# tongdaxu/VQ-VAE-from-Gaussian-VAE

Measured on AMD Instinct MI355X. Metric: images/sec encode+quantize+decode, 256x256, codebook 2^16, higher is better.
Workload: dtype f32

## Files before the change

include/gqhip.h:

```cpp
#ifndef GQHIP_H_
#define GQHIP_H_

#include <stdint.h>

#ifdef __cplusplus
extern "C" {
#endif

#define GQHIP_ABI_VERSION 8

typedef int64_t gqhip_gnstat_t;
#define GQHIP_GNSTAT_WORDS 8

typedef enum gqhip_status {
  GQHIP_OK = 0,
  GQHIP_ERR_INVALID_ARG = 1,
  GQHIP_ERR_WORKSPACE = 2,
  GQHIP_ERR_LAUNCH = 3,
  GQHIP_ERR_NO_DEVICE = 4
} gqhip_status;

int gqhip_abi_version(void);
const char *gqhip_status_string(int status);
int gqhip_last_hip_error(void);

#define GQHIP_FILTER_AUTO 0
#define GQHIP_FILTER_FP32 1
#define GQHIP_FILTER_BF16 2
#define GQHIP_FILTER_MIXED 3
int gqhip_set_filter(int kind);
int gqhip_get_filter(void);

int gqhip_debug_plan(int64_t rows, int64_t n, int64_t dim, int64_t *out8);


int64_t gqhip_workspace_bytes(int64_t rows, int64_t n, int64_t dim);

int64_t gqhip_cb_cache_bytes(int64_t n, int64_t dim);
int gqhip_grid_search_applies(int64_t n, int64_t dim);
int gqhip_cb_cache_degenerate(const void *cb_cache, int64_t n, int64_t dim);

int gq_scores_f32(const float *mu, const float *sd, const float *cb, float *out,
                  int64_t dim, int64_t rows, int64_t n, double beta,
                  void *stream);

int gq_argmax_f32(const float *mu, const float *sd, const float *logsd_or_null,
                  const float *cb, int64_t *idx, float *zhat_or_null,
                  int64_t dim, int64_t rows, int64_t n, double beta,
                  void *workspace, int64_t workspace_bytes,
                  void *cb_cache_or_null, int64_t cb_cache_bytes, void *stream);

#define GQHIP_LAYOUT_BCHW 0
#define GQHIP_LAYOUT_BLC 1
#define GQHIP_GROUP_STRIDED 0
#define GQHIP_GROUP_CONTIGUOUS 1
int gq_quantize_z_f32(const float *z, const float *noise_or_null, const float *cb,
                      int64_t *idx, float *zhat_or_null, float *zhat_noquant_or_null,
                      float *mu_out_or_null, float *sd_out_or_null, int64_t B,
                      int64_t L, int64_t c, int64_t dim, int64_t n, int layout,
                      int grouping, double lv_min, double lv_max, double beta,
                      void *workspace, int64_t workspace_bytes,
                      void *cb_cache_or_null, int64_t cb_cache_bytes, void *stream);

int gq_quantize_z_gauss_f32(const float *z, const float *noise, const float *cb, int64_t *idx, float *zhat,
                            float *zhat_quant_or_null, float *zhat_noquant, float *sd_out_or_null, void *scalars_out, double *lam_state, int64_t B,
                            int64_t L, int64_t c, int64_t dim, int64_t n, int layout, int grouping, double lv_min,
                            double lv_max, double beta, int use_ste, double log2n, double tolerance, double lam_factor,
                            double lam_lo, double lam_hi, int lam_max_decreases, void *workspace, int64_t workspace_bytes,
                            void *cb_cache_or_null, int64_t cb_cache_bytes, void *stream);

int gq_gauss_train_f32(const float *z, const float *noise, float *zhat, float *sd_out_or_null, float *kl2row, void *scalars_out,
                       double *lam_state, int64_t B, int64_t L, int64_t c, int64_t dim, int layout, int grouping, double lv_min,
                       double lv_max, double log2n, double tolerance, double lam_factor, double lam_lo, double lam_hi,
                       int lam_max_decreases, double loss_divisor, void *stream);

int gq_gauss_backward_f32(const float *z, const float *noise, const float *g_zhat_or_null, const float *g_sd_or_null,
                          const float *g_kl_or_null, const double *lam_before, float *grad_z, int64_t B, int64_t L, int64_t c,
                          int64_t dim, int layout, int grouping, double lv_min, double lv_max, double log2n, double tolerance,
                          double loss_divisor, void *stream);

int gq_dequant_f32(const int64_t *idx, const float *cb, float *zhat, int64_t B,
                   int64_t L, int64_t K, int64_t dim, int64_t n, int layout,
                   int grouping, void *stream);

int vq_argmin_f32(const float *z, const float *emb, int64_t *idx,
                  float *zq_or_null, int64_t dim, int64_t rows, int64_t n,
                  void *workspace, int64_t workspace_bytes,
                  void *cb_cache_or_null, int64_t cb_cache_bytes, void *stream);

int vq_quantize_z_f32(const float *z, const float *emb, int64_t *idx, float *zq, float *loss2_or_null, int64_t B, int64_t L,
                      int64_t c, int64_t dim, int64_t n, int layout, double beta, int legacy, void *workspace,
                      int64_t workspace_bytes, void *cb_cache_or_null, int64_t cb_cache_bytes, void *stream);

int lfq_pack_f32(const float *x, int64_t *idx, float *q_or_null, int64_t rows,
                 int64_t nbits, void *stream);
int lfq_unpack_f32(const int64_t *idx, float *q, int64_t rows, int64_t nbits,
                   void *stream);

int fsq_quantize_f32(const float *z, const int32_t *levels_host, int64_t nlev, float *zhat,
                     int32_t *idx, int64_t rows, void *stream);
int fsq_dequant_f32(const int32_t *idx, const int32_t *levels_host, int64_t nlev, float *zhat,
                    int64_t rows, void *stream);

#define GQHIP_LAYOUT_NCHW 0
#define GQHIP_LAYOUT_NHWC 1
int gn_silu_f32(const float *x, const float *gamma, const float *beta,
                const float *pre_bias_or_null, float *y, int64_t B, int64_t C, int64_t HW,
                int64_t groups, double eps, int apply_silu, int layout, gqhip_gnstat_t *stats_ws,
                void *stream);
int add_bias_f32(const float *a, const float *b, const float *bias_or_null, float *y, int64_t B,
                 int64_t C, int64_t HW, int layout, void *stream);

int add_bias_stats_f32(const float *a, const float *b, const float *bias_or_null, float *y, int64_t B,
                       int64_t C, int64_t HW, int64_t groups, gqhip_gnstat_t *stats_out, void *stream);

int gn_apply_f32(const float *x, const float *gamma, const float *beta, float *y, int64_t B, int64_t C,
                 int64_t HW, int64_t groups, double eps, int apply_silu, const gqhip_gnstat_t *stats, void *stream);

int gqhip_checksum_tensors(const void *table_dev, int64_t count, uint64_t *sums_dev, void *stream);

int gqhip_stats_prezeroed(int on);

int conv3x3_cin_small_f32(const float *x, const float *wk, const float *bias_or_null, float *y, int64_t *stats_out_or_null,
                          int64_t B, int64_t H, int64_t W, int64_t Cin, int64_t Cout, int64_t groups_out, void *stream);

int conv3x3_f32(const float *x, const float *gamma_or_null, const float *beta_or_null, const float *pre_bias_or_null,
                const gqhip_gnstat_t *stats_or_null, int64_t groups_in, double eps, int apply_silu, const float *wk,
                const float *bias_or_null, float *y, int64_t B, int64_t H, int64_t W, int64_t Cin, int64_t Cout, void *stream);

int upsample2x_nhwc_f32(const float *x, float *y, int64_t B, int64_t H, int64_t W, int64_t C,
                        void *stream);

int wino_in_nhwc_f32(const float *x, float *V, int64_t B, int64_t H, int64_t W, int64_t C, void *stream);
int wino_out_nhwc_f32(const float *M, float *y, int64_t B, int64_t H, int64_t W, int64_t C, float mscale, void *stream);

int wino_in_nhwc_f16x3(const float *x, void *V3, int64_t B, int64_t H, int64_t W, int64_t C, int tile, float scale,
                       void *stream);
int wino_in_nhwc_f16x2(const float *x, void *V2, int64_t B, int64_t H, int64_t W, int64_t C, int tile, float scale,
                       void *stream);
int wino_gemm_f16x2(const void *V2, const void *Wf, float *M, int64_t P, int64_t tiles, int64_t Cin, int64_t Cout,
                    void *stream);
int conv3x3_gn_f16x3(const float *x, const float *gamma, const float *beta, const float *pre_bias_or_null,
                     const gqhip_gnstat_t *stats_in, int64_t groups_in, double eps, int apply_silu, float scale, const void *Wf,
                     const float *bias_or_null, const float *res_or_null, float *y, gqhip_gnstat_t *stats_out_or_null, int64_t B,
                     int64_t H, int64_t W, int64_t Cin, int64_t Cout, int64_t groups_out, float mscale, void *stream);
int conv1x1_f16x3(const float *x, const float *pre_bias_or_null, const void *Wf, const float *scales_dev_or_null, float scale,
                  float mscale, const float *bias_or_null, const float *res_or_null, float *y, gqhip_gnstat_t *stats_out_or_null, int64_t B, int64_t HW,
                  int64_t Cin, int64_t Cout, int64_t groups_out, void *stream);
int conv3x3s2_f16x3(const float *x, const void *Wf, const float *scales_dev_or_null, float scale, float mscale,
                    const float *bias_or_null, float *y, gqhip_gnstat_t *stats_out_or_null, int64_t B, int64_t Hin, int64_t Win,
                    int64_t Cin, int64_t Cout, int64_t groups_out, void *stream);
int upconv2x_f16x3(const float *x, const void *Wf, const float *scales_dev_or_null, float scale, float mscale,
                   const float *bias_or_null, float *y, gqhip_gnstat_t *stats_out_or_null, int64_t B, int64_t H, int64_t W,
                   int64_t Cin, int64_t Cout, int64_t groups_out, void *stream);
int conv3x3_gn_small_f32(const float *x, const float *gamma, const float *beta, const float *pre_bias_or_null,
                         const gqhip_gnstat_t *stats_in, int64_t groups_in, double eps, int apply_silu, const float *w_ohwi,
                         const float *bias_or_null, float *y, int64_t B, int64_t H, int64_t W, int64_t Cin, int64_t Cout,
                         void *stream);
int wino_in_gn_nhwc_f16x3(const float *x, const float *gamma, const float *beta, const float *pre_bias_or_null,
                          const gqhip_gnstat_t *stats, void *V3, int64_t B, int64_t H, int64_t W, int64_t C, int64_t groups,
                          double eps, int apply_silu, int tile, float scale, void *stream);
int wino_in_gn_nhwc_f16x2(const float *x, const float *gamma, const float *beta, const float *pre_bias_or_null,
                          const gqhip_gnstat_t *stats, void *V2, int64_t B, int64_t H, int64_t W, int64_t C, int64_t groups,
                          double eps, int apply_silu, int tile, float scale, void *stream);

int wino4_in_nhwc_f32(const float *x, float *V, int64_t B, int64_t H, int64_t W, int64_t C, void *stream);
int wino4_out_nhwc_f32(const float *M, float *y, int64_t B, int64_t H, int64_t W, int64_t C, float mscale, void *stream);

int wino_out_res_nhwc_f32(const float *M, const float *res, const float *bias_or_null, float *y, gqhip_gnstat_t *stats_out,
                          int64_t B, int64_t H, int64_t W, int64_t C, int64_t groups, int tile, float mscale,
                          void *stream);

int gn_stats_f32(const float *x, const float *pre_bias_or_null, int64_t B, int64_t C, int64_t HW, int64_t groups,
                 gqhip_gnstat_t *stats_out, void *stream);

int wino_in_gn_nhwc_f32(const float *x, const float *gamma, const float *beta, const float *pre_bias_or_null,
                        const gqhip_gnstat_t *stats, float *V, int64_t B, int64_t H, int64_t W, int64_t C,
                        int64_t groups, double eps, int apply_silu, void *stream);
int wino4_in_gn_nhwc_f32(const float *x, const float *gamma, const float *beta, const float *pre_bias_or_null,
                         const gqhip_gnstat_t *stats, float *V, int64_t B, int64_t H, int64_t W, int64_t C,
                         int64_t groups, double eps, int apply_silu, void *stream);

int attn_split_qkv_f16x3(const float *qkv, void *Q3, void *K3, void *V3, int64_t B, int64_t L, int64_t C, float sq, float sv,
                         void *stream);
int attn_softmax_split_f16x3(const float *S, void *P3, int64_t rows, int64_t L, float factor, void *stream);
int f16_scales_from_gn_stats(const gqhip_gnstat_t *stats, int64_t n_bg, double amp, double u_scale, float *scales_out,
                             void *stream);

int gq_index_histogram(const int64_t *idx, int64_t count, int64_t n,
                       int32_t *hist, void *stream);
int gq_indices_to_u16(const int64_t *idx, uint16_t *out, int64_t count,
                      void *stream);
int gq_indices_from_u16(const uint16_t *in, int64_t *idx, int64_t count,
                        void *stream);

int64_t gq_step_record_workspace_bytes(int64_t B, int64_t per_image);
int gq_step_record_f32(const float *x, const float *x_rec, const int64_t *idx, int32_t *rec, int64_t B, int64_t per_image,
                       int64_t n_idx, void *workspace_zeroed, int64_t workspace_bytes, void *stream);

int64_t gq_ssim_workspace_bytes(int64_t B, int64_t C, int64_t H, int64_t W);
int gq_ssim_f32(const float *x, const float *x_rec, int64_t B, int64_t C, int64_t H, int64_t W, int layout, int zero_mean,
                float *ssim_out_or_null, float *msssim_out_or_null, void *workspace_zeroed, int64_t workspace_bytes, void *stream);
int64_t gq_step_record_ssim_workspace_bytes(int64_t B, int64_t C, int64_t H, int64_t W);
int gq_step_record_ssim_f32(const float *x, const float *x_rec, const int64_t *idx, int32_t *rec, int64_t B, int64_t C, int64_t H,
                            int64_t W, int layout, int64_t n_idx, void *workspace_zeroed, int64_t workspace_bytes, void *stream);

int64_t gq_mha_workspace_bytes(int64_t B, int64_t L, int64_t E, int64_t H);
int gq_mha_fwd_f32(const float *qkv, float *out, int64_t B, int64_t L, int64_t E, int64_t H, void *workspace, void *stream);

int gqhip_profile_enable(int on);
int gqhip_profile_reserve(int pairs);
int gqhip_profile_collect(int *launches_host, double *total_ms_host);

int gqhip_debug_enable(int on);
int gqhip_debug_counters(const void *workspace, int64_t *fallback_rows_host,
                         int64_t *reranked_halftiles_host);
int gqhip_debug_grid(const void *workspace, const void *cb_cache_or_null, int64_t *out4_host);
#ifdef __cplusplus
}
#endif
#endif
```

vq-vae-from-gaussian-vae_amd/csrc/gq_conv3.h:

```cpp
#pragma once
#include <type_traits>

#include "gq_common.h"
#include "gq_epilogue.h"
#include "gq_stats.h"
#include "gq_wino_gemm.h"

namespace gqhip {

constexpr int kC3TH = 8, kC3TW = 32;
constexpr int kC3PH = kC3TH + 2, kC3PW = kC3TW + 2;
constexpr int kC3Pix = kC3PH * kC3PW;
constexpr int kC3RS = 48;
constexpr int kC3Plane = kC3PH * kC3RS * 32;
constexpr int kC3Buf = 2 * kC3Plane;
constexpr int kC3Pieces = kC3Pix * 4;
constexpr int kC3Loads = (kC3Pieces + 255) / 256;

__device__ __forceinline__ int conv3_lds_off(int R, int x, int half) {
  return (R * kC3RS + x) * 32 + 16 * (half ^ ((x >> 3) & 1));
}

struct Conv3Params {
  const _Float16 *Xs;
  const _Float16 *Wf;
  const float *bias;
  const float *res;
  float *y;
  int64_t *stats;
  int H, W, nch, cpg;
  int cout, nnb;
  int tiles_x, tiles_y;
  long ntiles;
  long tiles_per_xcd;
  float mscale;
};

struct Conv3Tile {
  long b;
  int y0, x0, nb;
};
__device__ __forceinline__ bool conv3_tile(const Conv3Params &p, Conv3Tile &t, long vb = blockIdx.x) {
  const long k = vb >> 3;
  t.nb = (int)(k % p.nnb);
  const long tile = (long)(vb & 7) * p.tiles_per_xcd + k / p.nnb;
  if (tile >= p.ntiles) return false;
  const int tx = (int)(tile % p.tiles_x);
  const long t2 = tile / p.tiles_x;
  t.b = t2 / p.tiles_y;
  t.y0 = (int)(t2 % p.tiles_y) * kC3TH;
  t.x0 = tx * kC3TW;
  return true;
}

__device__ __forceinline__ void conv3_tap(const unsigned char *A, int dy, const f16x8 (&bq)[4], f32x16 (&acc)[4][2]) {
#pragma unroll
  for (int rr = 0; rr < 4; ++rr) {
#if defined(GQHIP_ABL) && (GQHIP_ABL & 256)
    const f16x8 ah = *reinterpret_cast<const f16x8 *>(A + dy * kC3RS * 32);
    const f16x8 al = ah;
#else
    const f16x8 ah = *reinterpret_cast<const f16x8 *>(A + (rr + dy) * kC3RS * 32);
    const f16x8 al = *reinterpret_cast<const f16x8 *>(A + (rr + dy) * kC3RS * 32 + kC3Plane);
#endif
#pragma unroll
    for (int j = 0; j < 2; ++j) {
      acc[rr][j] = __builtin_amdgcn_mfma_f32_32x32x16_f16(ah, bq[2 * j], acc[rr][j], 0, 0, 0);
      acc[rr][j] = __builtin_amdgcn_mfma_f32_32x32x16_f16(ah, bq[2 * j + 1], acc[rr][j], 0, 0, 0);
      acc[rr][j] = __builtin_amdgcn_mfma_f32_32x32x16_f16(al, bq[2 * j], acc[rr][j], 0, 0, 0);
    }
  }
}

template <int COUT>
__device__ __forceinline__ void conv3_epilogue(const Conv3Params &p, const Conv3Tile &t, const f32x16 (&acc)[4][2], unsigned char *sA,
                                               int64_t *red, int wave, int wm, int wn) {
  constexpr int cout = COUT;
  const int lane = __lane_id(), tid = wave * 64 + lane;
  const int n = wn * 64 + 4 * (lane & 15);
  float *stage = reinterpret_cast<float *>(sA + wave * kEpiWaveBytes);
  f32x4 pb = {0.f, 0.f, 0.f, 0.f};
  if (p.bias) {
#pragma unroll
    for (int e = 0; e < 4; ++e) pb[e] = p.bias[t.nb * 128 + n + e];
  }
  const long o = ((t.b * p.H + t.y0 + 4 * wm) * p.W + t.x0 + (lane >> 4)) * cout + t.nb * 128 + n;
  const long slice = (long)p.W * cout;
  StatPartial st;
  if (!p.stats) {
    if (p.res) epi_store<3, false>(acc, stage, lane, p.y, p.res, o, slice, 4 * cout, p.mscale, pb, st);
    else epi_store<2, false>(acc, stage, lane, p.y, nullptr, o, slice, 4 * cout, p.mscale, pb, st);
    return;
  }
  if (p.res) epi_store<3, true>(acc, stage, lane, p.y, p.res, o, slice, 4 * cout, p.mscale, pb, st);
  else epi_store<2, true>(acc, stage, lane, p.y, nullptr, o, slice, 4 * cout, p.mscale, pb, st);
  stat_partial_flush(red + kStatWords * (n / p.cpg), st);
  __syncthreads();
  const int gpb = 128 / p.cpg, groups = cout / p.cpg;
  if (tid < kStatWords * gpb) stat_flush_word(p.stats + kStatWords * (t.b * groups + t.nb * gpb) + tid, red[tid]);
}

#define GQ_C3_ZERO_ACC(acc)                                                                                         \
  _Pragma("unroll") for (int rr = 0; rr < 4; ++rr) _Pragma("unroll") for (int j = 0; j < 2; ++j) acc[rr][j] =       \
      f32x16{0.f, 0.f, 0.f, 0.f, 0.f, 0.f, 0.f, 0.f, 0.f, 0.f, 0.f, 0.f, 0.f, 0.f, 0.f, 0.f}

struct Conv3GnParams {
  Conv3Params c;
  const float *x;
  const float *gamma, *beta, *pre_bias;
  const int64_t *stats_in;
  int cin, cpg_in;
  double eps;
  float scale;
};

#ifdef GQHIP_CLOCK_STAMPS
__device__ unsigned long long g_c3_stamps[4 * 8192];
#endif
template <int SILU, int COUT>
__global__ __launch_bounds__(256, 2) void conv3x3_gn_f16x3_kernel(const Conv3GnParams pp) {
  typedef _Float16 f16x4 __attribute__((ext_vector_type(4)));
  const Conv3Params &p = pp.c;
  __shared__ __attribute__((aligned(16))) unsigned char sA[2 * kC3Buf];
  __shared__ int64_t red[kStatWords * 32];
  __shared__ __attribute__((aligned(16))) float sAff[2][512];
  const int tid = threadIdx.x, lane = tid & 63, wave = __builtin_amdgcn_readfirstlane(tid >> 6);
  const int c = lane & 31, h = lane >> 5, wm = wave >> 1, wn = wave & 1;
#ifdef GQHIP_CLOCK_STAMPS
  const unsigned long long st_r0 = __builtin_amdgcn_s_memrealtime();
#endif
  Conv3Tile t;
  if (!conv3_tile(p, t)) return;
  const int H = p.H, W = p.W, cin = pp.cin;
  red[tid] = 0;
  {
    const int groups = cin / pp.cpg_in;
    const double n = (double)pp.cpg_in * (double)H * (double)W;
    for (int ch = tid; ch < cin; ch += 256) {
      const int g = ch / pp.cpg_in;
      double st_s, st_ss;
      stat_load(pp.stats_in + kStatWords * (t.b * groups + g), st_s, st_ss);
      const double mean = st_s / n;
      double var = st_ss / n - mean * mean;
      var = var > 0.0 ? var : 0.0;
      const double rstd = 1.0 / sqrt(var + pp.eps);
      const double pbk = pp.pre_bias ? (double)pp.pre_bias[ch] : 0.0;
      sAff[0][ch] = (float)(rstd * (double)pp.gamma[ch]);
      sAff[1][ch] = (float)((double)pp.beta[ch] + (pbk - mean) * rstd * (double)pp.gamma[ch]);
    }
  }
  const int w = tid & 3, qs = tid >> 2;
  int goff[kC3Loads];
  unsigned inb = 0;
#pragma unroll
  for (int i = 0; i < kC3Loads; ++i) {
    int q = qs + 64 * i;
    q = q < kC3Pix ? q : kC3Pix - 1;
    const int R = q / kC3PW, px = q % kC3PW;
    const int gy = t.y0 - 1 + R, gx = t.x0 - 1 + px;
    const bool in = gy >= 0 && gy < H && gx >= 0 && gx < W;
    const int cy = gy < 0 ? 0 : (gy >= H ? H - 1 : gy), cx = gx < 0 ? 0 : (gx >= W ? W - 1 : gx);
    goff[i] = (cy * W + cx) * cin + 4 * w;
    inb |= (unsigned)(in ? 1 : 0) << i;
  }
  const float *xb = pp.x + t.b * (long)H * W * cin;
  f32x4 st[3];
  auto issue = [&](int i, int chunk) { st[i % 3] = *reinterpret_cast<const f32x4 *>(xb + goff[i] + chunk * 16); };
  auto convert = [&](int i, int chunk, int buf) {
    const int q = qs + 64 * i;
    if (q >= kC3Pix) return;
    const f32x4 a4 = *reinterpret_cast<const f32x4 *>(&sAff[0][chunk * 16 + 4 * w]);
    const f32x4 sh4 = *reinterpret_cast<const f32x4 *>(&sAff[1][chunk * 16 + 4 * w]);
    const f32x4 v = gn_act<SILU>(st[i % 3], a4, sh4) * (((inb >> i) & 1) ? pp.scale : 0.f);
    f16x4 hi, lo;
#pragma unroll
    for (int e = 0; e < 4; ++e) {
      hi[e] = (_Float16)v[e];
      lo[e] = (_Float16)(v[e] - (float)hi[e]);
    }
    const int off = buf * kC3Buf + conv3_lds_off(q / kC3PW, q % kC3PW, w >> 1) + 8 * (w & 1);
    *reinterpret_cast<f16x4 *>(&sA[off]) = hi;
    *reinterpret_cast<f16x4 *>(&sA[off + kC3Plane]) = lo;
  };

  f32x16 acc[4][2];
  GQ_C3_ZERO_ACC(acc);
  int aoff[3];
#pragma unroll
  for (int dx = 0; dx < 3; ++dx) aoff[dx] = conv3_lds_off(4 * wm, c + dx, h);
  const unsigned char *wbase = reinterpret_cast<const unsigned char *>(p.Wf) + (4 * t.nb + 2 * wn) * 128 * 16;
  const int wl = lane * 16;
  const long wstep = (long)p.nnb * (512 * 16);
  f16x8 bs[3][4];
  auto load_b = [&](int ks, f16x8 (&dst)[4]) {
    const unsigned char *s = wbase + ks * wstep;
#pragma unroll
    for (int k = 0; k < 4; ++k) dst[k] = *reinterpret_cast<const f16x8 *>(s + k * 1024 + wl);
  };
  const int nks = p.nch * 9;
  load_b(0, bs[0]);
  load_b(1, bs[1]);
  __syncthreads();
  for (int i0 = 0; i0 < kC3Loads; i0 += 3) {
#pragma unroll
    for (int i = 0; i < 3; ++i) issue(i0 + i, 0);
#pragma unroll
    for (int i = 0; i < 3; ++i) convert(i0 + i, 0, 0);
  }
  __syncthreads();

#ifdef GQHIP_CLOCK_STAMPS
  const unsigned long long st_r1 = __builtin_amdgcn_s_memrealtime();
#endif
  for (int chunk = 0; chunk < p.nch; ++chunk) {
    const bool more = chunk + 1 < p.nch;
    const unsigned char *A = sA + (chunk & 1) * kC3Buf;
    const int nbuf = (chunk + 1) & 1;
#pragma unroll
    for (int tap = 0; tap < 9; ++tap) {
      const int ks = chunk * 9 + tap;
#if !(defined(GQHIP_ABL) && (GQHIP_ABL & 128))
      load_b(ks + 2 < nks ? ks + 2 : nks - 1, bs[(tap + 2) % 3]);
#endif
      conv3_tap(A + aoff[tap % 3], tap / 3, bs[tap % 3], acc);
#if !(defined(GQHIP_ABL) && (GQHIP_ABL & 64))
      if (more) {
        if (tap >= 3) convert(tap - 3, chunk + 1, nbuf);
        if (tap < kC3Loads) issue(tap, chunk + 1);
      }
#endif
      __builtin_amdgcn_sched_barrier(0);
    }
    __syncthreads();
  }
#ifdef GQHIP_CLOCK_STAMPS
  const unsigned long long st_r2 = __builtin_amdgcn_s_memrealtime();
#endif
#if defined(GQHIP_ABL) && (GQHIP_ABL & 512)
  if (acc[0][0][0] == 12345.678f)
#endif
  conv3_epilogue<COUT>(p, t, acc, sA, red, wave, wm, wn);
#ifdef GQHIP_CLOCK_STAMPS
  if (tid == 0 && blockIdx.x < 8192) {
    unsigned long long *o = g_c3_stamps + 4 * blockIdx.x;
    o[0] = st_r0;
    o[1] = __builtin_amdgcn_s_memrealtime();
    o[2] = ((st_r1 - st_r0) << 32) | (st_r2 - st_r0);
    o[3] = ((unsigned long long)__builtin_amdgcn_s_getreg((31 << 11) | 20) << 32) | (unsigned)__builtin_amdgcn_s_getreg((31 << 11) | 4);
  }
#endif
}



struct Conv1Params {
  Conv3Params c;
  const float *x;
  const float *pre_bias;
  const float *scales_dev;
  float scale;
  int cin;
};

template <int COUT>
__global__ __launch_bounds__(256, 2) void conv1x1_f16x3_kernel(const Conv1Params pp) {
  typedef _Float16 f16x4 __attribute__((ext_vector_type(4)));
  Conv3Params p = pp.c;
  constexpr int kPlane = 256 * 32, kChunk = 2 * kPlane, kStage = 2 * kChunk;
  __shared__ __attribute__((aligned(16))) unsigned char sA[2 * kStage];
  __shared__ int64_t red[kStatWords * 32];
  const int tid = threadIdx.x, lane = tid & 63, wave = __builtin_amdgcn_readfirstlane(tid >> 6);
  const int c = lane & 31, h = lane >> 5, wm = wave >> 1, wn = wave & 1;
  Conv3Tile t;
  if (!conv3_tile(p, t)) return;
  red[tid] = 0;
  const float scale = pp.scales_dev ? pp.scales_dev[0] : pp.scale;
  if (pp.scales_dev) p.mscale = pp.scales_dev[1];
  const int cin = pp.cin, nst = cin / 32;
  const int w8 = tid & 7, r0 = tid >> 3;
  const float *xb = pp.x + ((t.b * p.H + t.y0) * 32L + r0) * cin + 4 * w8;
  const float *pbp = pp.pre_bias ? pp.pre_bias + 4 * w8 : nullptr;
  f32x4 pb4 = {0.f, 0.f, 0.f, 0.f};
  const int loff = (w8 >> 2) * kChunk + r0 * 32 + 16 * (((w8 >> 1) & 1) ^ ((r0 >> 3) & 1)) + 8 * (w8 & 1);
  f32x4 st[8];
  auto issue = [&](int stage) {
#pragma unroll
    for (int i = 0; i < 8; ++i) st[i] = *reinterpret_cast<const f32x4 *>(xb + (long)(32 * i) * cin + stage * 32);
  };
  auto convert = [&](int i, int buf) {
    const f32x4 v = (st[i] + pb4) * scale;
    f16x4 hi, lo;
#pragma unroll
    for (int e = 0; e < 4; ++e) {
      hi[e] = (_Float16)v[e];
      lo[e] = (_Float16)(v[e] - (float)hi[e]);
    }
    unsigned char *d = sA + buf * kStage + loff + i * (32 * 32);
    *reinterpret_cast<f16x4 *>(d) = hi;
    *reinterpret_cast<f16x4 *>(d + kPlane) = lo;
  };
  f32x16 acc[4][2];
  GQ_C3_ZERO_ACC(acc);
  const int aoff = (4 * wm) * 1024 + c * 32 + 16 * (h ^ ((c >> 3) & 1));
  const unsigned char *wbase = reinterpret_cast<const unsigned char *>(p.Wf) + (4 * t.nb + 2 * wn) * 128 * 16;
  const int wl = lane * 16;
  const long wstep = (long)p.nnb * (512 * 16);
  f16x8 b0[4], b1[4];
  auto load_b = [&](int ks, f16x8 (&dst)[4]) {
    const unsigned char *s = wbase + ks * wstep;
#pragma unroll
    for (int k = 0; k < 4; ++k) dst[k] = *reinterpret_cast<const f16x8 *>(s + k * 1024 + wl);
  };
  auto kstep = [&](const unsigned char *A, const f16x8 (&bq)[4]) {
#pragma unroll
    for (int rr = 0; rr < 4; ++rr) {
      const f16x8 ah = *reinterpret_cast<const f16x8 *>(A + aoff + rr * 1024);
      const f16x8 al = *reinterpret_cast<const f16x8 *>(A + aoff + rr * 1024 + kPlane);
#pragma unroll
      for (int j = 0; j < 2; ++j) {
        acc[rr][j] = __builtin_amdgcn_mfma_f32_32x32x16_f16(ah, bq[2 * j], acc[rr][j], 0, 0, 0);
        acc[rr][j] = __builtin_amdgcn_mfma_f32_32x32x16_f16(ah, bq[2 * j + 1], acc[rr][j], 0, 0, 0);
        acc[rr][j] = __builtin_amdgcn_mfma_f32_32x32x16_f16(al, bq[2 * j], acc[rr][j], 0, 0, 0);
      }
    }
  };
  const int nks = 2 * nst;
  load_b(0, b0);
  issue(0);
  if (pbp) pb4 = *reinterpret_cast<const f32x4 *>(pbp);
#pragma unroll
  for (int i = 0; i < 8; ++i) convert(i, 0);
  __syncthreads();
  for (int s = 0; s < nst; ++s) {
    const bool more = s + 1 < nst;
    const unsigned char *A = sA + (s & 1) * kStage;
    const int nbuf = (s + 1) & 1;
    load_b(2 * s + 1, b1);
    if (more) issue(s + 1);
    kstep(A, b0);
    __builtin_amdgcn_sched_barrier(0);
    load_b(2 * s + 2 < nks ? 2 * s + 2 : nks - 1, b0);
    kstep(A + kChunk, b1);
    if (more) {
      if (pbp) pb4 = *reinterpret_cast<const f32x4 *>(pbp + (s + 1) * 32);
#pragma unroll
      for (int i = 0; i < 8; ++i) convert(i, nbuf);
    }
    __builtin_amdgcn_sched_barrier(0);
    __syncthreads();
  }
  conv3_epilogue<COUT>(p, t, acc, sA, red, wave, wm, wn);
}

struct Conv3S2Params {
  Conv3Params c;
  const float *x;
  const float *scales_dev;
  float scale;
  int cin, Hin, Win;
};

template <int COUT>
__global__ __launch_bounds__(256, 2) void conv3x3s2_f16x3_kernel(const Conv3S2Params pp) {
  typedef _Float16 f16x4 __attribute__((ext_vector_type(4)));
  Conv3Params p = pp.c;
  __shared__ __attribute__((aligned(16))) unsigned char sA[2 * kC3Buf];
  __shared__ int64_t red[kStatWords * 32];
  const int tid = threadIdx.x, lane = tid & 63, wave = __builtin_amdgcn_readfirstlane(tid >> 6);
  const int c = lane & 31, h = lane >> 5, wm = wave >> 1, wn = wave & 1;
  Conv3Tile t;
  if (!conv3_tile(p, t)) return;
  red[tid] = 0;
  const float scale = pp.scales_dev ? pp.scales_dev[0] : pp.scale;
  if (pp.scales_dev) p.mscale = pp.scales_dev[1];
  const int cin = pp.cin, nch = p.nch, Hin = pp.Hin, Win = pp.Win;
  constexpr int PR = kC3TH + 1, PC = kC3TW + 1, NP = 5;
  const int w = tid & 3, qs = tid >> 2;
  const float *xb = pp.x + t.b * (long)Hin * Win * cin + 4 * w;
  int goff[NP], loff[NP];
  unsigned inb = 0;
  auto setup_phase = [&](int a, int b) {
    inb = 0;
#pragma unroll
    for (int i = 0; i < NP; ++i) {
      const int q = qs + 64 * i;
      const int qq = q < PR * PC ? q : PR * PC - 1;
      const int R = qq / PC, X = qq % PC;
      const int gy = 2 * (t.y0 + R) + a, gx = 2 * (t.x0 + X) + b;
      const bool in = gy < Hin && gx < Win;
      const int cy = gy < Hin ? gy : Hin - 1, cx = gx < Win ? gx : Win - 1;
      goff[i] = (cy * Win + cx) * cin;
      loff[i] = q < PR * PC ? conv3_lds_off(R, X, w >> 1) + 8 * (w & 1) : -1;
      inb |= (unsigned)(in ? 1 : 0) << i;
    }
  };
  f32x4 st[NP];
  auto issue = [&](int chunk) {
#pragma unroll
    for (int i = 0; i < NP; ++i) st[i] = *reinterpret_cast<const f32x4 *>(xb + goff[i] + chunk * 16);
  };
  auto commit = [&](int buf) {
#pragma unroll
    for (int i = 0; i < NP; ++i) {
      if (loff[i] < 0) continue;
      const f32x4 v = st[i] * (((inb >> i) & 1) ? scale : 0.f);
      f16x4 hi, lo;
#pragma unroll
      for (int e = 0; e < 4; ++e) {
        hi[e] = (_Float16)v[e];
        lo[e] = (_Float16)(v[e] - (float)hi[e]);
      }
      unsigned char *d = sA + buf * kC3Buf + loff[i];
      *reinterpret_cast<f16x4 *>(d) = hi;
      *reinterpret_cast<f16x4 *>(d + kC3Plane) = lo;
    }
  };
  f32x16 acc[4][2];
  GQ_C3_ZERO_ACC(acc);
  int aoff[2];
#pragma unroll
  for (int dx = 0; dx < 2; ++dx) aoff[dx] = conv3_lds_off(4 * wm, c + dx, h);
  const unsigned char *wbase = reinterpret_cast<const unsigned char *>(p.Wf) + (4 * t.nb + 2 * wn) * 128 * 16;
  const int wl = lane * 16;
  const long wstep = (long)p.nnb * (512 * 16);
  f16x8 bq[4], bn[4];
  auto load_b = [&](int ks, f16x8 (&dst)[4]) {
    const unsigned char *s = wbase + ks * wstep;
#pragma unroll
    for (int k = 0; k < 4; ++k) dst[k] = *reinterpret_cast<const f16x8 *>(s + k * 1024 + wl);
  };
  const int nks = 9 * nch;
  int ks = 0, unit = 0;
  load_b(0, bq);
  setup_phase(0, 0);
  issue(0);
  commit(0);
  __syncthreads();
  auto run_unit = [&](auto nt_tag, auto a_tag, auto b_tag, int chunk) {
    constexpr int NT = decltype(nt_tag)::value, PA = decltype(a_tag)::value, PB = decltype(b_tag)::value;
    const bool last_chunk = chunk + 1 >= nch;
    const bool more = !(last_chunk && PA == 1 && PB == 1);
    if (more) {
      if (last_chunk) setup_phase(PB == 1 ? 1 : PA, PB == 1 ? 0 : 1);
      issue(last_chunk ? 0 : chunk + 1);
    }
    const unsigned char *A = sA + (unit & 1) * kC3Buf;
#pragma unroll
    for (int ti = 0; ti < NT; ++ti) {
      const int ddy = (PA == 0 && PB == 0) ? ti / 2 : (PA == 0 && PB == 1) ? ti : 0;
      const int ddx = (PA == 0 && PB == 0) ? ti % 2 : (PA == 1 && PB == 0) ? ti : 0;
      load_b(ks + 1 < nks ? ks + 1 : ks, bn);
      conv3_tap(A + aoff[ddx], ddy, bq, acc);
#pragma unroll
      for (int k = 0; k < 4; ++k) bq[k] = bn[k];
      ++ks;
      __builtin_amdgcn_sched_barrier(0);
    }
    if (more) commit((unit + 1) & 1);
    ++unit;
    __syncthreads();
  };
  using I0 = std::integral_constant<int, 0>; using I1 = std::integral_constant<int, 1>;
  using I2 = std::integral_constant<int, 2>; using I4 = std::integral_constant<int, 4>;
  for (int chunk = 0; chunk < nch; ++chunk) run_unit(I4{}, I0{}, I0{}, chunk);
  for (int chunk = 0; chunk < nch; ++chunk) run_unit(I2{}, I0{}, I1{}, chunk);
  for (int chunk = 0; chunk < nch; ++chunk) run_unit(I2{}, I1{}, I0{}, chunk);
  for (int chunk = 0; chunk < nch; ++chunk) run_unit(I1{}, I1{}, I1{}, chunk);
  conv3_epilogue<COUT>(p, t, acc, sA, red, wave, wm, wn);
}

struct Upconv2Params {
  Conv3Params c;
  const float *x;
  const float *scales_dev;
  float scale;
  int cin;
};

template <int COUT>
__global__ __launch_bounds__(256, 2) void upconv2x_f16x3_kernel(const Upconv2Params pp) {
  typedef _Float16 f16x4 __attribute__((ext_vector_type(4)));
  Conv3Params p = pp.c;
  __shared__ __attribute__((aligned(16))) unsigned char sA[2 * kC3Buf];
  __shared__ int64_t red[kStatWords * 32];
  const int tid = threadIdx.x, lane = tid & 63, wave = __builtin_amdgcn_readfirstlane(tid >> 6);
  const int c = lane & 31, h = lane >> 5, wm = wave >> 1, wn = wave & 1;
  Conv3Tile t;
  if (!conv3_tile(p, t)) return;
  const int pa = (int)blockIdx.y >> 1, pb = (int)blockIdx.y & 1;
  red[tid] = 0;
  const float scale = pp.scales_dev ? pp.scales_dev[0] : pp.scale;
  if (pp.scales_dev) p.mscale = pp.scales_dev[1];
  const int cin = pp.cin, nch = p.nch, H = p.H, W = p.W;
  constexpr int PR = kC3TH + 1, PC = kC3TW + 1, NP = 5;
  const int w = tid & 3, qs = tid >> 2;
  const float *xb = pp.x + t.b * (long)H * W * cin + 4 * w;
  int goff[NP], loff[NP];
  unsigned inb = 0;
#pragma unroll
  for (int i = 0; i < NP; ++i) {
    const int q = qs + 64 * i;
    const int qq = q < PR * PC ? q : PR * PC - 1;
    const int R = qq / PC, X = qq % PC;
    const int gy = t.y0 + R + pa - 1, gx = t.x0 + X + pb - 1;
// ... 164 lines not shown
```

vq-vae-from-gaussian-vae_amd/csrc/gq_epilogue.h:

```cpp
#pragma once
#include "gq_common.h"
#include "gq_stats.h"

namespace gqhip {

constexpr int kEpiWaveBytes = 32 * 64 * 4;

__device__ __forceinline__ void epi_wave_sync() {
  __builtin_amdgcn_fence(__ATOMIC_RELEASE, "wavefront");
  __builtin_amdgcn_wave_barrier();
  __builtin_amdgcn_fence(__ATOMIC_ACQUIRE, "wavefront");
}

__device__ __forceinline__ void epi_transpose(const f32x16 (&a)[2], float *stage, int lane, f32x4 (&out)[8]) {
  const int c = lane & 31, h = lane >> 5;
  epi_wave_sync();
#pragma unroll
  for (int j = 0; j < 2; ++j)
#pragma unroll
    for (int r = 0; r < 16; ++r) stage[((r & 3) + 8 * (r >> 2) + 4 * h) * 64 + 32 * j + c] = a[j][r];
  epi_wave_sync();
  const f32x4 *s = reinterpret_cast<const f32x4 *>(stage) + (lane >> 4) * 16 + (lane & 15);
#pragma unroll
  for (int i = 0; i < 8; ++i) out[i] = s[64 * i];
}

template <int MODE, bool STATS>
__device__ __forceinline__ void epi_store(const f32x16 (&acc)[4][2], float *stage, int lane, float *y, const float *res,
                                          long o, long slice, long step, float mscale, f32x4 bias, StatPartial &st) {
#pragma unroll
  for (int rr = 0; rr < 4; ++rr) {
    __builtin_amdgcn_sched_barrier(0);
    const long orr = o + rr * slice;
    f32x4 rv[8];
#pragma unroll
    for (int i = 0; i < 8; ++i)
      rv[i] = MODE == 3 ? *reinterpret_cast<const f32x4 *>(res + orr + i * step) : f32x4{0.f, 0.f, 0.f, 0.f};
    f32x4 v[8];
    epi_transpose(acc[rr], stage, lane, v);
#pragma unroll
    for (int i = 0; i < 8; ++i) {
      f32x4 w = v[i];
      w = w * mscale + bias;
      if (MODE >= 2) w = w + rv[i];
      *reinterpret_cast<f32x4 *>(y + orr + i * step) = w;
      if (STATS) stat_partial_add_vec(st, w);
    }
  }
}

}
```

vq-vae-from-gaussian-vae_amd/csrc/gqhip_unet.hip:

```cpp
#include "gqhip.h"

#include <hip/hip_ext.h>
#include <hip/hip_runtime.h>

#include <cstdlib>
#include <cstring>

#include "gqhip_internal.h"
#include "gq_unet_aux.h"
#include "gq_wino_gemm.h"
#include "gq_conv3.h"
#include "gq_conv_f32.h"
#include "gq_attn.h"

using namespace gqhip;

namespace {
thread_local int g_stats_prezeroed = 0;
inline hipError_t stats_zero(void *p, size_t bytes, hipStream_t st) {
  return g_stats_prezeroed ? hipSuccess : hipMemsetAsync(p, 0, bytes, st);
}
}

extern "C" {
// ... 154 lines not shown
  if (!V2 || !Wf || !M) return GQHIP_ERR_INVALID_ARG;
  WinoGemm2Params wp{};
  wp.V2 = static_cast<const _Float16 *>(V2); wp.Wf = static_cast<const _Float16 *>(Wf); wp.M = M; wp.tiles = tiles;
  wp.cin = (int)Cin; wp.cout = (int)Cout;
  const WinoGemmTiling tiling = wino_gemm_tiling(Cin, Cout);
  const long rows = tiling == WinoGemmTiling::k128x256 ? 128 : 256, cols = tiling == WinoGemmTiling::k256x128 ? 128 : 256;
  wp.nnb = (int)(Cout / cols);
  wp.mtiles = tiles / rows; wp.ntile_total = P * wp.mtiles; wp.tiles_per_xcd = (wp.ntile_total + 7) / 8;
  const long blocks = 8 * wp.tiles_per_xcd * wp.nnb;
  if (blocks > 0x7fffffffL) return GQHIP_ERR_INVALID_ARG;
  hipStream_t st = static_cast<hipStream_t>(stream);
  switch (tiling) {
    case WinoGemmTiling::k128x256: hipLaunchKernelGGL(wino_gemm_f16x2_k64_kernel<1>, dim3((unsigned)blocks), dim3(256), 0, st, wp); break;
    case WinoGemmTiling::k256x256: hipLaunchKernelGGL(wino_gemm_f16x2_k64_kernel<2>, dim3((unsigned)blocks), dim3(512), 0, st, wp); break;
    case WinoGemmTiling::k256x128: hipLaunchKernelGGL(wino_gemm_f16x2_kernel, dim3((unsigned)blocks), dim3(256), 0, st, wp); break;
  }
  return check_launch();
}

int gn_stats_f32(const float *x, const float *pre_bias_or_null, int64_t B, int64_t C, int64_t HW, int64_t groups,
                 int64_t *stats_out, void *stream) {
  if (B < 0 || C < 1 || HW < 1 || groups < 1 || C % groups != 0) return GQHIP_ERR_INVALID_ARG;
  if (B == 0) return GQHIP_OK;
  if (!x || !stats_out) return GQHIP_ERR_INVALID_ARG;
  const int64_t cpg = C / groups;
  if (cpg % 4 != 0 || 256 % (C / 4) != 0 || groups > 64) return GQHIP_ERR_INVALID_ARG;
  hipStream_t st = static_cast<hipStream_t>(stream);
  if (stats_zero(stats_out, sizeof(int64_t) * kStatWords * B * groups, st) != hipSuccess) return check_launch();
  const int slabs = nhwc_slabs(C, HW);
  return launch(gn_stats_nhwc_kernel, dim3((unsigned)(B * slabs)), dim3(256), 0, st, x, pre_bias_or_null, stats_out,
                (int)C, (long)HW, (int)cpg, slabs);
}

static int wino_in_gn_impl(int tile, int f16, const float *x, const float *gamma, const float *beta,
                           const float *pre_bias_or_null, const int64_t *stats, void *V, int64_t B, int64_t H, int64_t W,
                           int64_t C, int64_t groups, double eps, int apply_silu, float scale, void *stream) {
  if (B < 0 || H < tile || W < tile || H % tile || W % tile || C < 4 || C % 4 != 0 || groups < 1 || C % groups != 0 ||
      (C / groups) % 4 != 0 || !(scale > 0.f))
    return GQHIP_ERR_INVALID_ARG;
  if (B == 0) return GQHIP_OK;
  if (!x || !gamma || !beta || !stats || !V) return GQHIP_ERR_INVALID_ARG;
  const int vw = (tile == 4 && f16 != 0) ? 2 : 4;
  const long tiles = (long)(B * (H / tile) * (W / tile)), total = tiles * (C / vw);
  long blocks = (total + 255) / 256;
  if (blocks > 32768) blocks = 32768;
  hipStream_t st = static_cast<hipStream_t>(stream);
#define GQ_WGN(K, ...)                                                                                                  \
  hipLaunchKernelGGL((K<__VA_ARGS__>), dim3((unsigned)blocks), dim3(256), 0, st, x, gamma, beta, pre_bias_or_null, stats, \
                     V, (int)H, (int)W, (int)(C / vw), (int)(C / groups), eps, tiles, total, scale)
  if (tile == 4) {
    if (apply_silu) {
      if (f16 == 2) GQ_WGN(wino4_in_gn_nhwc_kernel, 1, 2, 2); else if (f16 == 1) GQ_WGN(wino4_in_gn_nhwc_kernel, 1, 1, 2);
      else GQ_WGN(wino4_in_gn_nhwc_kernel, 1, 0, 4);
    } else {
      if (f16 == 2) GQ_WGN(wino4_in_gn_nhwc_kernel, 0, 2, 2); else if (f16 == 1) GQ_WGN(wino4_in_gn_nhwc_kernel, 0, 1, 2);
      else GQ_WGN(wino4_in_gn_nhwc_kernel, 0, 0, 4);
    }
  } else {
    if (apply_silu) {
      if (f16 == 2) GQ_WGN(wino_in_gn_nhwc_kernel, 1, 2); else if (f16 == 1) GQ_WGN(wino_in_gn_nhwc_kernel, 1, 1);
      else GQ_WGN(wino_in_gn_nhwc_kernel, 1, 0);
    } else {
      if (f16 == 2) GQ_WGN(wino_in_gn_nhwc_kernel, 0, 2); else if (f16 == 1) GQ_WGN(wino_in_gn_nhwc_kernel, 0, 1);
      else GQ_WGN(wino_in_gn_nhwc_kernel, 0, 0);
    }
  }
#undef GQ_WGN
  return check_launch();
}

int wino_in_gn_nhwc_f32(const float *x, const float *gamma, const float *beta, const float *pre_bias_or_null,
                        const int64_t *stats, float *V, int64_t B, int64_t H, int64_t W, int64_t C, int64_t groups,
                        double eps, int apply_silu, void *stream) {
  return wino_in_gn_impl(2, 0, x, gamma, beta, pre_bias_or_null, stats, V, B, H, W, C, groups, eps, apply_silu, 1.0f, stream);
}

int wino4_in_gn_nhwc_f32(const float *x, const float *gamma, const float *beta, const float *pre_bias_or_null,
                         const int64_t *stats, float *V, int64_t B, int64_t H, int64_t W, int64_t C, int64_t groups,
                         double eps, int apply_silu, void *stream) {
  return wino_in_gn_impl(4, 0, x, gamma, beta, pre_bias_or_null, stats, V, B, H, W, C, groups, eps, apply_silu, 1.0f, stream);
}

int wino_in_gn_nhwc_f16x3(const float *x, const float *gamma, const float *beta, const float *pre_bias_or_null,
                          const int64_t *stats, void *V3, int64_t B, int64_t H, int64_t W, int64_t C, int64_t groups,
                          double eps, int apply_silu, int tile, float scale, void *stream) {
  if (tile != 2 && tile != 4) return GQHIP_ERR_INVALID_ARG;
  return wino_in_gn_impl(tile, 1, x, gamma, beta, pre_bias_or_null, stats, V3, B, H, W, C, groups, eps, apply_silu, scale,
                         stream);
}

int wino_in_gn_nhwc_f16x2(const float *x, const float *gamma, const float *beta, const float *pre_bias_or_null,
                          const int64_t *stats, void *V2, int64_t B, int64_t H, int64_t W, int64_t C, int64_t groups,
                          double eps, int apply_silu, int tile, float scale, void *stream) {
  if (tile != 2 && tile != 4) return GQHIP_ERR_INVALID_ARG;
  return wino_in_gn_impl(tile, 2, x, gamma, beta, pre_bias_or_null, stats, V2, B, H, W, C, groups, eps, apply_silu, scale,
                         stream);
}

static bool conv3_groups_ok(int64_t Cout, int64_t groups_out) {
  if (groups_out < 1 || Cout % groups_out != 0) return false;
  const int64_t cpg = Cout / groups_out;
  return cpg % 4 == 0 && 128 % cpg == 0;
}

static void conv3_fill(Conv3Params &cp, const void *Wf, const float *bias, const float *res, float *y, int64_t *stats, int64_t B,
                       int64_t H, int64_t W, int64_t Cin, int64_t Cout, int64_t groups_out, float mscale) {
  cp.Wf = static_cast<const _Float16 *>(Wf);
  cp.bias = bias; cp.res = res; cp.y = y; cp.stats = stats;
  cp.H = (int)H; cp.W = (int)W; cp.nch = (int)(Cin / 16); cp.cpg = stats ? (int)(Cout / groups_out) : 4;
  cp.cout = (int)Cout; cp.nnb = (int)(Cout / 128);
  cp.tiles_x = (int)(W / kC3TW); cp.tiles_y = (int)(H / kC3TH);
  cp.ntiles = (long)B * cp.tiles_x * cp.tiles_y;
  cp.tiles_per_xcd = (cp.ntiles + 7) / 8;
  cp.mscale = mscale;
}

int conv3x3_gn_f16x3(const float *x, const float *gamma, const float *beta, const float *pre_bias_or_null,
                     const int64_t *stats_in, int64_t groups_in, double eps, int apply_silu, float scale, const void *Wf,
                     const float *bias_or_null, const float *res_or_null, float *y, int64_t *stats_out_or_null, int64_t B,
                     int64_t H, int64_t W, int64_t Cin, int64_t Cout, int64_t groups_out, float mscale, void *stream) {
  if (B < 0 || H < kC3TH || W < kC3TW || H % kC3TH || W % kC3TW || Cin < 32 || Cin % 32 != 0 || Cin > 512 || (Cout != 128 && Cout != 256) ||
      H * W > (1 << 22) || groups_in < 1 || Cin % groups_in != 0 || !(scale > 0.f))
    return GQHIP_ERR_INVALID_ARG;
  if (stats_out_or_null && !conv3_groups_ok(Cout, groups_out)) return GQHIP_ERR_INVALID_ARG;
  if (B == 0) return GQHIP_OK;
  if (!x || !gamma || !beta || !stats_in || !Wf || !y) return GQHIP_ERR_INVALID_ARG;
  hipStream_t st = static_cast<hipStream_t>(stream);
  if (stats_out_or_null && stats_zero(stats_out_or_null, sizeof(int64_t) * kStatWords * B * groups_out, st) != hipSuccess)
    return check_launch();
  Conv3GnParams gp{};
  Conv3Params &cp = gp.c;
  cp.Xs = nullptr;
  conv3_fill(cp, Wf, bias_or_null, res_or_null, y, stats_out_or_null, B, H, W, Cin, Cout, groups_out, mscale);
  gp.x = x; gp.gamma = gamma; gp.beta = beta; gp.pre_bias = pre_bias_or_null; gp.stats_in = stats_in;
  gp.cin = (int)Cin; gp.cpg_in = (int)(Cin / groups_in); gp.eps = eps; gp.scale = scale;
  const dim3 grid((unsigned)(8 * cp.tiles_per_xcd * cp.nnb));
  static const int env_dyn = getenv("GQHIP_C3_DYNLDS") ? atoi(getenv("GQHIP_C3_DYNLDS")) : 0;
  if (Cout == 128) {
    if (apply_silu) hipLaunchKernelGGL((conv3x3_gn_f16x3_kernel<1, 128>), grid, dim3(256), env_dyn, st, gp);
    else hipLaunchKernelGGL((conv3x3_gn_f16x3_kernel<0, 128>), grid, dim3(256), 0, st, gp);
  } else {
    if (apply_silu) hipLaunchKernelGGL((conv3x3_gn_f16x3_kernel<1, 256>), grid, dim3(256), 0, st, gp);
    else hipLaunchKernelGGL((conv3x3_gn_f16x3_kernel<0, 256>), grid, dim3(256), 0, st, gp);
  }
  return check_launch();
}

#ifdef GQHIP_CLOCK_STAMPS
extern "C" int gqhip_debug_c3_stamps(unsigned long long *out, int64_t words) {
  return hipMemcpyFromSymbol(out, HIP_SYMBOL(g_c3_stamps), sizeof(unsigned long long) * words) == hipSuccess ? 0 : 1;
}
#endif

int conv1x1_f16x3(const float *x, const float *pre_bias_or_null, const void *Wf, const float *scales_dev_or_null, float scale,
                  float mscale, const float *bias_or_null, const float *res_or_null, float *y, int64_t *stats_out_or_null, int64_t B, int64_t HW,
                  int64_t Cin, int64_t Cout, int64_t groups_out, void *stream) {
  if (B < 0 || HW < 256 || HW % 256 != 0 || Cin < 32 || Cin % 32 != 0 || (Cout != 128 && Cout != 256 && Cout != 512 && Cout != 1536) ||
      HW > (1 << 24) || (!scales_dev_or_null && !(scale > 0.f)))
    return GQHIP_ERR_INVALID_ARG;
  if (stats_out_or_null && !conv3_groups_ok(Cout, groups_out)) return GQHIP_ERR_INVALID_ARG;
  if (B == 0) return GQHIP_OK;
  if (!x || !Wf || !y) return GQHIP_ERR_INVALID_ARG;
  hipStream_t st = static_cast<hipStream_t>(stream);
  if (stats_out_or_null && stats_zero(stats_out_or_null, sizeof(int64_t) * kStatWords * B * groups_out, st) != hipSuccess)
    return check_launch();
  Conv1Params gp{};
  Conv3Params &cp = gp.c;
  conv3_fill(cp, Wf, bias_or_null, res_or_null, y, stats_out_or_null, B, HW / 32, 32, Cin, Cout, groups_out, mscale);
  cp.nch = (int)(Cin / 16);
  gp.x = x; gp.pre_bias = pre_bias_or_null; gp.scales_dev = scales_dev_or_null; gp.scale = scale; gp.cin = (int)Cin;
  const dim3 grid((unsigned)(8 * cp.tiles_per_xcd * cp.nnb));
  if (Cout == 128) hipLaunchKernelGGL(conv1x1_f16x3_kernel<128>, grid, dim3(256), 0, st, gp);
  else if (Cout == 256) hipLaunchKernelGGL(conv1x1_f16x3_kernel<256>, grid, dim3(256), 0, st, gp);
  else if (Cout == 512) hipLaunchKernelGGL(conv1x1_f16x3_kernel<512>, grid, dim3(256), 0, st, gp);
  else hipLaunchKernelGGL(conv1x1_f16x3_kernel<1536>, grid, dim3(256), 0, st, gp);
  return check_launch();
}

int conv3x3s2_f16x3(const float *x, const void *Wf, const float *scales_dev_or_null, float scale, float mscale,
                    const float *bias_or_null, float *y, int64_t *stats_out_or_null, int64_t B, int64_t Hin, int64_t Win,
                    int64_t Cin, int64_t Cout, int64_t groups_out, void *stream) {
  if (B < 0 || Hin < 2 * kC3TH || Win < 2 * kC3TW || Hin % (2 * kC3TH) || Win % (2 * kC3TW) || Cin < 16 || Cin % 16 != 0 ||
      (Cout != 128 && Cout != 256 && Cout != 512) || Hin * Win > (1 << 24) || (!scales_dev_or_null && !(scale > 0.f)))
    return GQHIP_ERR_INVALID_ARG;
  if (stats_out_or_null && !conv3_groups_ok(Cout, groups_out)) return GQHIP_ERR_INVALID_ARG;
  if (B == 0) return GQHIP_OK;
  if (!x || !Wf || !y) return GQHIP_ERR_INVALID_ARG;
  hipStream_t st = static_cast<hipStream_t>(stream);
  if (stats_out_or_null && stats_zero(stats_out_or_null, sizeof(int64_t) * kStatWords * B * groups_out, st) != hipSuccess)
    return check_launch();
  Conv3S2Params gp{};
  Conv3Params &cp = gp.c;
  conv3_fill(cp, Wf, bias_or_null, nullptr, y, stats_out_or_null, B, Hin / 2, Win / 2, Cin, Cout, groups_out, mscale);
  gp.x = x; gp.scales_dev = scales_dev_or_null; gp.scale = scale; gp.cin = (int)Cin; gp.Hin = (int)Hin; gp.Win = (int)Win;
  const dim3 grid((unsigned)(8 * cp.tiles_per_xcd * cp.nnb));
  if (Cout == 128) hipLaunchKernelGGL(conv3x3s2_f16x3_kernel<128>, grid, dim3(256), 0, st, gp);
  else if (Cout == 256) hipLaunchKernelGGL(conv3x3s2_f16x3_kernel<256>, grid, dim3(256), 0, st, gp);
  else hipLaunchKernelGGL(conv3x3s2_f16x3_kernel<512>, grid, dim3(256), 0, st, gp);
  return check_launch();
}

int upconv2x_f16x3(const float *x, const void *Wf, const float *scales_dev_or_null, float scale, float mscale,
                   const float *bias_or_null, float *y, int64_t *stats_out_or_null, int64_t B, int64_t H, int64_t W,
                   int64_t Cin, int64_t Cout, int64_t groups_out, void *stream) {
  if (B < 0 || H < kC3TH || W < kC3TW || H % kC3TH || W % kC3TW || Cin < 16 || Cin % 16 != 0 ||
      (Cout != 128 && Cout != 256 && Cout != 512) || H * W > (1 << 22) || (!scales_dev_or_null && !(scale > 0.f)))
    return GQHIP_ERR_INVALID_ARG;
  if (stats_out_or_null && !conv3_groups_ok(Cout, groups_out)) return GQHIP_ERR_INVALID_ARG;
  if (B == 0) return GQHIP_OK;
  if (!x || !Wf || !y) return GQHIP_ERR_INVALID_ARG;
  hipStream_t st = static_cast<hipStream_t>(stream);
  if (stats_out_or_null && stats_zero(stats_out_or_null, sizeof(int64_t) * kStatWords * B * groups_out, st) != hipSuccess)
    return check_launch();
  Upconv2Params gp{};
  Conv3Params &cp = gp.c;
  conv3_fill(cp, Wf, bias_or_null, nullptr, y, stats_out_or_null, B, H, W, Cin, Cout, groups_out, mscale);
  gp.x = x; gp.scales_dev = scales_dev_or_null; gp.scale = scale; gp.cin = (int)Cin;
  const dim3 grid((unsigned)(8 * cp.tiles_per_xcd * cp.nnb), 4);
  if (Cout == 128) hipLaunchKernelGGL(upconv2x_f16x3_kernel<128>, grid, dim3(256), 0, st, gp);
  else if (Cout == 256) hipLaunchKernelGGL(upconv2x_f16x3_kernel<256>, grid, dim3(256), 0, st, gp);
  else hipLaunchKernelGGL(upconv2x_f16x3_kernel<512>, grid, dim3(256), 0, st, gp);
  return check_launch();
}

int conv3x3_gn_small_f32(const float *x, const float *gamma, const float *beta, const float *pre_bias_or_null,
                         const int64_t *stats_in, int64_t groups_in, double eps, int apply_silu, const float *w_ohwi,
                         const float *bias_or_null, float *y, int64_t B, int64_t H, int64_t W, int64_t Cin, int64_t Cout,
                         void *stream) {
  if (B < 0 || H < 16 || W < 16 || H % 16 || W % 16 || Cin < 32 || Cin % 32 != 0 || Cin > 512 || Cout < 1 || Cout > 4 ||
      groups_in < 1 || Cin % groups_in != 0 || B * (H / 16) * (W / 16) > 0x7fffffffL)
    return GQHIP_ERR_INVALID_ARG;
  if (B == 0) return GQHIP_OK;
  if (!x || !gamma || !beta || !stats_in || !w_ohwi || !y) return GQHIP_ERR_INVALID_ARG;
  hipStream_t st = static_cast<hipStream_t>(stream);
  const dim3 grid((unsigned)(B * (H / 16) * (W / 16)));
  const int cpg = (int)(Cin / groups_in);
#define GQ_CS(S, CO)                                                                                                      \
  hipLaunchKernelGGL((conv3x3_gn_small_kernel<S, CO>), grid, dim3(256), 0, st, x, gamma, beta, pre_bias_or_null, stats_in, \
                     w_ohwi, bias_or_null, y, (int)H, (int)W, (int)Cin, cpg, eps)
#define GQ_CS2(CO) do { if (apply_silu) GQ_CS(1, CO); else GQ_CS(0, CO); } while (0)
  switch (Cout) {
    case 1: GQ_CS2(1); break;
    case 2: GQ_CS2(2); break;
    case 3: GQ_CS2(3); break;
    default: GQ_CS2(4); break;
  }
#undef GQ_CS2
#undef GQ_CS
  return check_launch();
}

int conv3x3_cin_small_f32(const float *x, const float *wk, const float *bias_or_null, float *y, int64_t *stats_out_or_null,
                          int64_t B, int64_t H, int64_t W, int64_t Cin, int64_t Cout, int64_t groups_out, void *stream) {
  if (B < 0 || H < 8 || W < 32 || H % 8 || W % 32 || Cin < 1 || Cin > 4 || Cout != 128 || B * (H / 8) * (W / 32) > 0x7fffffffL)
    return GQHIP_ERR_INVALID_ARG;
  if (stats_out_or_null && groups_out != 32) return GQHIP_ERR_INVALID_ARG;
  if (B == 0) return GQHIP_OK;
  if (!x || !wk || !y) return GQHIP_ERR_INVALID_ARG;
  hipStream_t st = static_cast<hipStream_t>(stream);
  if (stats_out_or_null && stats_zero(stats_out_or_null, sizeof(int64_t) * kStatWords * B * 32, st) != hipSuccess)
    return check_launch();
  ConvInParams cp{};
  cp.x = x; cp.wk = wk; cp.bias = bias_or_null; cp.y = y; cp.stats = stats_out_or_null; cp.H = (int)H; cp.W = (int)W;
  const dim3 grid((unsigned)(B * (H / 8) * (W / 32)));
  switch (Cin) {
    case 1: hipLaunchKernelGGL(conv3x3_cin_small_kernel<1>, grid, dim3(256), 0, st, cp); break;
    case 2: hipLaunchKernelGGL(conv3x3_cin_small_kernel<2>, grid, dim3(256), 0, st, cp); break;
    case 3: hipLaunchKernelGGL(conv3x3_cin_small_kernel<3>, grid, dim3(256), 0, st, cp); break;
    default: hipLaunchKernelGGL(conv3x3_cin_small_kernel<4>, grid, dim3(256), 0, st, cp); break;
  }
  return check_launch();
}

int conv3x3_f32(const float *x, const float *gamma_or_null, const float *beta_or_null, const float *pre_bias_or_null,
                const int64_t *stats_or_null, int64_t groups_in, double eps, int apply_silu, const float *wk,
                const float *bias_or_null, float *y, int64_t B, int64_t H, int64_t W, int64_t Cin, int64_t Cout, void *stream) {
  if (B < 0 || H < 1 || W < 1 || Cin < 8 || Cout < 4 || Cout % 4 != 0 || B * H * ((W + 31) / 32) > 0x7fffffffL)
    return GQHIP_ERR_INVALID_ARG;
  if (B == 0) return GQHIP_OK;
  if (!x || !wk || !y) return GQHIP_ERR_INVALID_ARG;
  const bool gn = stats_or_null != nullptr;
  if (gn && (!gamma_or_null || !beta_or_null || groups_in < 1 || Cin % groups_in != 0 || Cin > 1024)) return GQHIP_ERR_INVALID_ARG;
  hipStream_t st = static_cast<hipStream_t>(stream);
  ConvF32Params cp{};
  cp.x = x; cp.gamma = gamma_or_null; cp.beta = beta_or_null; cp.pre_bias = pre_bias_or_null; cp.stats = stats_or_null;
  cp.wk = wk; cp.bias = bias_or_null; cp.y = y;
  cp.H = (int)H; cp.W = (int)W; cp.Cin = (int)Cin; cp.Cout = (int)Cout; cp.cpg = gn ? (int)(Cin / groups_in) : 1; cp.eps = eps;
  const unsigned segs = (unsigned)(B * H * ((W + 31) / 32));
  if (Cin % 64 == 0) {
    const dim3 grid(segs, (unsigned)((Cout + 31) / 32));
    if (gn && apply_silu) hipLaunchKernelGGL((conv3x3_f32_ksplit_kernel<true, 1>), grid, dim3(256), 0, st, cp);
    else if (gn) hipLaunchKernelGGL((conv3x3_f32_ksplit_kernel<true, 0>), grid, dim3(256), 0, st, cp);
    else hipLaunchKernelGGL((conv3x3_f32_ksplit_kernel<false, 0>), grid, dim3(256), 0, st, cp);
    return check_launch();
  }
  if (gn) return GQHIP_ERR_INVALID_ARG;
  switch (Cin) {
    case 8: hipLaunchKernelGGL((conv3x3_f32_nsplit_kernel<8>), dim3(segs), dim3(256), 0, st, cp); break;
    case 16: hipLaunchKernelGGL((conv3x3_f32_nsplit_kernel<16>), dim3(segs), dim3(256), 0, st, cp); break;
    case 32: hipLaunchKernelGGL((conv3x3_f32_nsplit_kernel<32>), dim3(segs), dim3(256), 0, st, cp); break;
    default: return GQHIP_ERR_INVALID_ARG;
  }
  return check_launch();
}

int wino_out_nhwc_f32(const float *M, float *y, int64_t B, int64_t H, int64_t W, int64_t C, float mscale, void *stream) {
  if (B < 0 || H < 2 || W < 2 || H % 2 || W % 2 || C < 4 || C % 4 != 0) return GQHIP_ERR_INVALID_ARG;
  if (B == 0) return GQHIP_OK;
  if (!M || !y) return GQHIP_ERR_INVALID_ARG;
  const long tiles = (long)(B * (H / 2) * (W / 2)), total = tiles * (C / 4);
  long blocks = (total + 255) / 256;
  if (blocks > 16384) blocks = 16384;
  return launch(wino_out_nhwc_kernel, dim3((unsigned)blocks), dim3(256), 0, static_cast<hipStream_t>(stream), M, y,
                (int)H, (int)W, (int)(C / 4), tiles, total, mscale);
}

int wino4_in_nhwc_f32(const float *x, float *V, int64_t B, int64_t H, int64_t W, int64_t C, void *stream) {
  if (B < 0 || H < 4 || W < 4 || H % 4 || W % 4 || C < 4 || C % 4 != 0) return GQHIP_ERR_INVALID_ARG;
  if (B == 0) return GQHIP_OK;
  if (!x || !V) return GQHIP_ERR_INVALID_ARG;
  const long tiles = (long)(B * (H / 4) * (W / 4)), total = tiles * (C / 4);
  long blocks = (total + 255) / 256;
  if (blocks > 16384) blocks = 16384;
  return launch(wino4_in_nhwc_kernel<0>, dim3((unsigned)blocks), dim3(256), 0, static_cast<hipStream_t>(stream), x,
                (void *)V, (int)H, (int)W, (int)(C / 4), tiles, total, 1.0f);
}

int wino4_out_nhwc_f32(const float *M, float *y, int64_t B, int64_t H, int64_t W, int64_t C, float mscale, void *stream) {
  if (B < 0 || H < 4 || W < 4 || H % 4 || W % 4 || C < 4 || C % 4 != 0) return GQHIP_ERR_INVALID_ARG;
// ... 117 lines not shown
```

vq-vae-from-gaussian-vae_amd/pit_hip/_lib.py:

```python
from __future__ import annotations

import ctypes
import threading
import math
import os
import subprocess
from typing import Optional, Tuple

import torch

_CSRC = os.path.normpath(os.path.join(os.path.dirname(os.path.abspath(__file__)), "..", "csrc"))
LIB_PATH = os.environ.get("GQHIP_LIB", os.path.join(_CSRC, "libgqhip.so"))

ABI_VERSION = 8
GNSTAT_WORDS = 8
GQHIP_LAYOUT = {"bchw": 0, "blc": 1}
GQHIP_GROUP_STRIDED = 0
GQHIP_GROUP_CONTIGUOUS = 1

_lib: Optional[ctypes.CDLL] = None

_vp = ctypes.c_void_p
_i64 = ctypes.c_int64
_SIGNATURES = {
    "gqhip_abi_version": (ctypes.c_int, []),
    "gqhip_status_string": (ctypes.c_char_p, [ctypes.c_int]),
    "gqhip_last_hip_error": (ctypes.c_int, []),
    "gqhip_workspace_bytes": (_i64, [_i64, _i64, _i64]),
    "gqhip_cb_cache_bytes": (_i64, [_i64, _i64]),
    "gqhip_grid_search_applies": (ctypes.c_int, [_i64, _i64]),
    "gqhip_cb_cache_degenerate": (ctypes.c_int, [_vp, _i64, _i64]),
    "gqhip_debug_grid": (ctypes.c_int, [_vp, _vp, ctypes.POINTER(_i64)]),
    "gqhip_set_filter": (ctypes.c_int, [ctypes.c_int]),
    "gqhip_get_filter": (ctypes.c_int, []),
    "gqhip_debug_plan": (ctypes.c_int, [_i64, _i64, _i64, ctypes.POINTER(_i64)]),
    "gq_scores_f32": (ctypes.c_int, [_vp, _vp, _vp, _vp, _i64, _i64, _i64, ctypes.c_double, _vp]),
    "gq_argmax_f32": (ctypes.c_int, [_vp, _vp, _vp, _vp, _vp, _vp, _i64, _i64, _i64, ctypes.c_double, _vp, _i64, _vp, _i64, _vp]),
    "gq_quantize_z_f32": (ctypes.c_int, [_vp, _vp, _vp, _vp, _vp, _vp, _vp, _vp, _i64, _i64, _i64, _i64, _i64,
                                         ctypes.c_int, ctypes.c_int, ctypes.c_double, ctypes.c_double,
                                         ctypes.c_double, _vp, _i64, _vp, _i64, _vp]),
    "gq_quantize_z_gauss_f32": (ctypes.c_int, [_vp, _vp, _vp, _vp, _vp, _vp, _vp, _vp, _vp, _vp, _i64, _i64, _i64, _i64, _i64,
                                               ctypes.c_int, ctypes.c_int, ctypes.c_double, ctypes.c_double, ctypes.c_double,
                                               ctypes.c_int, ctypes.c_double, ctypes.c_double, ctypes.c_double, ctypes.c_double,
                                               ctypes.c_double, ctypes.c_int, _vp, _i64, _vp, _i64, _vp]),
    "gq_gauss_train_f32": (ctypes.c_int, [_vp, _vp, _vp, _vp, _vp, _vp, _vp, _i64, _i64, _i64, _i64, ctypes.c_int, ctypes.c_int,
                                          ctypes.c_double, ctypes.c_double, ctypes.c_double, ctypes.c_double, ctypes.c_double,
                                          ctypes.c_double, ctypes.c_double, ctypes.c_int, ctypes.c_double, _vp]),
    "gq_gauss_backward_f32": (ctypes.c_int, [_vp, _vp, _vp, _vp, _vp, _vp, _vp, _i64, _i64, _i64, _i64, ctypes.c_int, ctypes.c_int,
                                             ctypes.c_double, ctypes.c_double, ctypes.c_double, ctypes.c_double, ctypes.c_double,
                                             _vp]),
    "vq_quantize_z_f32": (ctypes.c_int, [_vp, _vp, _vp, _vp, _vp, _i64, _i64, _i64, _i64, _i64, ctypes.c_int, ctypes.c_double,
                                         ctypes.c_int, _vp, _i64, _vp, _i64, _vp]),
    "gq_dequant_f32": (ctypes.c_int, [_vp, _vp, _vp, _i64, _i64, _i64, _i64, _i64, ctypes.c_int,
                                      ctypes.c_int, _vp]),
    "vq_argmin_f32": (ctypes.c_int, [_vp, _vp, _vp, _vp, _i64, _i64, _i64, _vp, _i64, _vp, _i64, _vp]),
    "lfq_pack_f32": (ctypes.c_int, [_vp, _vp, _vp, _i64, _i64, _vp]),
    "lfq_unpack_f32": (ctypes.c_int, [_vp, _vp, _i64, _i64, _vp]),
    "fsq_quantize_f32": (ctypes.c_int, [_vp, ctypes.POINTER(ctypes.c_int32), _i64, _vp, _vp, _i64, _vp]),
    "fsq_dequant_f32": (ctypes.c_int, [_vp, ctypes.POINTER(ctypes.c_int32), _i64, _vp, _i64, _vp]),
    "gn_silu_f32": (ctypes.c_int, [_vp, _vp, _vp, _vp, _vp, _i64, _i64, _i64, _i64, ctypes.c_double, ctypes.c_int,
                                   ctypes.c_int, _vp, _vp]),
    "add_bias_stats_f32": (ctypes.c_int, [_vp, _vp, _vp, _vp, _i64, _i64, _i64, _i64, _vp, _vp]),
    "gn_apply_f32": (ctypes.c_int, [_vp, _vp, _vp, _vp, _i64, _i64, _i64, _i64, ctypes.c_double, ctypes.c_int, _vp, _vp]),
    "wino_in_nhwc_f32": (ctypes.c_int, [_vp, _vp, _i64, _i64, _i64, _i64, _vp]),
    "wino4_in_nhwc_f32": (ctypes.c_int, [_vp, _vp, _i64, _i64, _i64, _i64, _vp]),
    "wino4_out_nhwc_f32": (ctypes.c_int, [_vp, _vp, _i64, _i64, _i64, _i64, ctypes.c_float, _vp]),
    "wino_out_res_nhwc_f32": (ctypes.c_int, [_vp, _vp, _vp, _vp, _vp, _i64, _i64, _i64, _i64, _i64, ctypes.c_int,
                                              ctypes.c_float, _vp]),
    "wino_in_nhwc_f16x3": (ctypes.c_int, [_vp, _vp, _i64, _i64, _i64, _i64, ctypes.c_int, ctypes.c_float, _vp]),
    "wino_in_nhwc_f16x2": (ctypes.c_int, [_vp, _vp, _i64, _i64, _i64, _i64, ctypes.c_int, ctypes.c_float, _vp]),
    "wino_gemm_f16x2": (ctypes.c_int, [_vp, _vp, _vp, _i64, _i64, _i64, _i64, _vp]),
    "upconv2x_f16x3": (ctypes.c_int, [_vp, _vp, _vp, ctypes.c_float, ctypes.c_float, _vp, _vp, _vp, _i64, _i64, _i64, _i64, _i64, _i64,
                                      _vp]),
    "attn_split_qkv_f16x3": (ctypes.c_int, [_vp, _vp, _vp, _vp, _i64, _i64, _i64, ctypes.c_float, ctypes.c_float, _vp]),
    "attn_softmax_split_f16x3": (ctypes.c_int, [_vp, _vp, _i64, _i64, ctypes.c_float, _vp]),
    "wino_in_gn_nhwc_f16x3": (ctypes.c_int, [_vp, _vp, _vp, _vp, _vp, _vp, _i64, _i64, _i64, _i64, _i64, ctypes.c_double,
                                              ctypes.c_int, ctypes.c_int, ctypes.c_float, _vp]),
    "wino_in_gn_nhwc_f16x2": (ctypes.c_int, [_vp, _vp, _vp, _vp, _vp, _vp, _i64, _i64, _i64, _i64, _i64, ctypes.c_double,
                                              ctypes.c_int, ctypes.c_int, ctypes.c_float, _vp]),
    "conv3x3_gn_f16x3": (ctypes.c_int, [_vp, _vp, _vp, _vp, _vp, _i64, ctypes.c_double, ctypes.c_int, ctypes.c_float, _vp,
                                         _vp, _vp, _vp, _vp, _i64, _i64, _i64, _i64, _i64, _i64, ctypes.c_float, _vp]),
    "conv1x1_f16x3": (ctypes.c_int, [_vp, _vp, _vp, _vp, ctypes.c_float, ctypes.c_float, _vp, _vp, _vp, _vp, _i64, _i64, _i64, _i64, _i64,
                                      _vp]),
    "conv3x3s2_f16x3": (ctypes.c_int, [_vp, _vp, _vp, ctypes.c_float, ctypes.c_float, _vp, _vp, _vp, _i64, _i64, _i64, _i64, _i64,
                                        _i64, _vp]),
    "conv3x3_gn_small_f32": (ctypes.c_int, [_vp, _vp, _vp, _vp, _vp, _i64, ctypes.c_double, ctypes.c_int, _vp, _vp, _vp, _i64, _i64,
                                             _i64, _i64, _i64, _vp]),
    "conv3x3_cin_small_f32": (ctypes.c_int, [_vp, _vp, _vp, _vp, _vp, _i64, _i64, _i64, _i64, _i64, _i64, _vp]),
    "conv3x3_f32": (ctypes.c_int, [_vp, _vp, _vp, _vp, _vp, _i64, ctypes.c_double, ctypes.c_int, _vp, _vp, _vp, _i64, _i64, _i64,
                                   _i64, _i64, _vp]),
    "gqhip_checksum_tensors": (ctypes.c_int, [_vp, _i64, _vp, _vp]),
    "gn_stats_f32": (ctypes.c_int, [_vp, _vp, _i64, _i64, _i64, _i64, _vp, _vp]),
    "wino_in_gn_nhwc_f32": (ctypes.c_int, [_vp, _vp, _vp, _vp, _vp, _vp, _i64, _i64, _i64, _i64, _i64, ctypes.c_double,
                                            ctypes.c_int, _vp]),
    "wino4_in_gn_nhwc_f32": (ctypes.c_int, [_vp, _vp, _vp, _vp, _vp, _vp, _i64, _i64, _i64, _i64, _i64, ctypes.c_double,
                                             ctypes.c_int, _vp]),
    "wino_out_nhwc_f32": (ctypes.c_int, [_vp, _vp, _i64, _i64, _i64, _i64, ctypes.c_float, _vp]),
    "f16_scales_from_gn_stats": (ctypes.c_int, [_vp, _i64, ctypes.c_double, ctypes.c_double, _vp, _vp]),
    "upsample2x_nhwc_f32": (ctypes.c_int, [_vp, _vp, _i64, _i64, _i64, _i64, _vp]),
    "add_bias_f32": (ctypes.c_int, [_vp, _vp, _vp, _vp, _i64, _i64, _i64, ctypes.c_int, _vp]),
    "gqhip_stats_prezeroed": (ctypes.c_int, [ctypes.c_int]),
    "gq_index_histogram": (ctypes.c_int, [_vp, _i64, _i64, _vp, _vp]),
    "gq_indices_to_u16": (ctypes.c_int, [_vp, _vp, _i64, _vp]),
    "gq_indices_from_u16": (ctypes.c_int, [_vp, _vp, _i64, _vp]),
    "gq_step_record_workspace_bytes": (_i64, [_i64, _i64]),
    "gq_step_record_f32": (ctypes.c_int, [_vp, _vp, _vp, _vp, _i64, _i64, _i64, _vp, _i64, _vp]),
    "gq_ssim_workspace_bytes": (_i64, [_i64, _i64, _i64, _i64]),
    "gq_ssim_f32": (ctypes.c_int, [_vp, _vp, _i64, _i64, _i64, _i64, ctypes.c_int, ctypes.c_int, _vp, _vp, _vp, _i64, _vp]),
    "gq_step_record_ssim_workspace_bytes": (_i64, [_i64, _i64, _i64, _i64]),
    "gq_step_record_ssim_f32": (ctypes.c_int, [_vp, _vp, _vp, _vp, _i64, _i64, _i64, _i64, ctypes.c_int, _i64, _vp, _i64, _vp]),
    "gq_mha_workspace_bytes": (_i64, [_i64, _i64, _i64, _i64]),
    "gq_mha_fwd_f32": (ctypes.c_int, [_vp, _vp, _i64, _i64, _i64, _i64, _vp, _vp]),
    "gqhip_profile_enable": (ctypes.c_int, [ctypes.c_int]),
    "gqhip_profile_reserve": (ctypes.c_int, [ctypes.c_int]),
    "gqhip_profile_collect": (ctypes.c_int, [ctypes.POINTER(ctypes.c_int), ctypes.POINTER(ctypes.c_double)]),
    "gqhip_debug_enable": (ctypes.c_int, [ctypes.c_int]),
    "gqhip_debug_counters": (ctypes.c_int, [_vp, ctypes.POINTER(_i64), ctypes.POINTER(_i64)]),
}
EXPORTED_SYMBOLS = tuple(_SIGNATURES)


class GqHipError(RuntimeError):
    pass


def build(force: bool = False) -> str:
    args = ["make", "-C", _CSRC, "-s", "-j4"]
    if force:
        args.append("-B")
    subprocess.check_call(args + ["libgqhip.so"])
    return LIB_PATH


def lib() -> ctypes.CDLL:
    global _lib
    if _lib is None:
        if not os.path.exists(LIB_PATH):
            raise GqHipError(
                f"{LIB_PATH} is missing: run `python -c 'import __graft_entry__ as g; g.build()'` "
                "(or `make -C vq-vae-from-gaussian-vae_amd/csrc`). There is no CPU fallback."
            )
        L = ctypes.CDLL(LIB_PATH)
        for name, (res, args) in _SIGNATURES.items():
            fn = getattr(L, name)
            fn.restype = res
            fn.argtypes = args
        if L.gqhip_abi_version() != ABI_VERSION:
            raise GqHipError("libgqhip.so ABI version mismatch")
        _lib = L
    return _lib


def _check(rc: int, what: str) -> None:
    if rc != 0:
        L = lib()
        raise GqHipError(f"{what}: {L.gqhip_status_string(rc).decode()} (hipError {L.gqhip_last_hip_error()})")


def _dev(t: torch.Tensor, dtype: torch.dtype, name: str) -> torch.Tensor:
    if not isinstance(t, torch.Tensor) or not t.is_cuda:
        raise GqHipError(f"{name} must be a tensor on a HIP device (got {getattr(t, 'device', type(t))}); "
                         "the HIP path has no CPU fallback")
    if t.dtype != dtype:
        raise GqHipError(f"{name} must be {dtype}, got {t.dtype}")
    return t if t.is_contiguous() else t.contiguous()


def _stream() -> int:
    return torch.cuda.current_stream().cuda_stream


def _ptr(t: Optional[torch.Tensor]) -> Optional[int]:
    return None if t is None else t.data_ptr()


class Workspace:

    def __init__(self) -> None:
        self.buf: Optional[torch.Tensor] = None
        self.cache_buf: Optional[torch.Tensor] = None
        self._cache_key = None
        self._cache_calls = 0
        self.no_search = False
        self._pinned = False

    def cache(self, n: int, dim: int, device) -> Tuple[Optional[int], int]:
        need = lib().gqhip_cb_cache_bytes(n, dim)
        if need <= 0 or self.no_search:
            return None, 0
        key = (n, dim, device)
        if self.cache_buf is None or self._cache_key != key or self.cache_buf.numel() < need:
            if torch.cuda.is_current_stream_capturing() or self._pinned:
                raise GqHipError("the codebook cache would have to be (re)allocated during / after a HIP graph capture that uses "
                                 "this Workspace: run a warm-up call of the same codebook shape before capturing")
            self.cache_buf = torch.zeros(need, dtype=torch.uint8, device=device)
            self._cache_key = key
            self._cache_calls = 0
        self._cache_calls += 1
        if self._cache_calls == 2 and lib().gqhip_grid_search_applies(n, dim) and not torch.cuda.is_current_stream_capturing():
            if lib().gqhip_cb_cache_degenerate(self.cache_buf.data_ptr(), n, dim) == 1:
                self.no_search = True
                return None, 0
        return self.cache_buf.data_ptr(), self.cache_buf.numel()

    def reserve(self, rows: int, n: int, dim: int, device) -> None:
        self.get(rows, n, dim, device)
        self.cache(n, dim, device)

    def get(self, rows: int, n: int, dim: int, device) -> Tuple[int, int]:
        need = lib().gqhip_workspace_bytes(rows, n, dim)
        if need < 0:
            raise GqHipError(f"unsupported shape rows={rows} n={n} dim={dim}")
        capturing = torch.cuda.is_current_stream_capturing()
        if self.buf is None or self.buf.numel() < need or self.buf.device != device:
            if capturing or self._pinned:
                raise GqHipError("workspace would have to grow during / after a HIP graph capture that uses it: "
                                 "run a warm-up call of the largest shape before capturing, or use a separate Workspace")
            self.buf = torch.empty(need, dtype=torch.uint8, device=device)
        if capturing:
            self._pinned = True
        return self.buf.data_ptr(), self.buf.numel()


def gq_scores(mu, sd, cb, out, beta: float = 1.0) -> None:
    mu, sd, cb = (_dev(t, torch.float32, n) for t, n in ((mu, "mu"), (sd, "std"), (cb, "codebook")))
    if not (out.is_cuda and out.dtype == torch.float32 and out.is_contiguous()):
        raise GqHipError("out must be a contiguous float32 HIP tensor")
    rows, dim = mu.shape
    n = cb.shape[0]
    if sd.shape != mu.shape or cb.shape[1] != dim or tuple(out.shape) != (rows, n):
        raise GqHipError("shape mismatch in gq_scores")
    with torch.cuda.device(mu.device):
        _check(lib().gq_scores_f32(mu.data_ptr(), sd.data_ptr(), cb.data_ptr(), out.data_ptr(), dim, rows, n,
                                   float(beta), _stream()), "gq_scores_f32")


# ... 331 lines not shown
                                 groups, float(eps), 1 if silu else 0, layout, ws.data_ptr(), _stream()), "gn_silu_f32")
    return y


def add_bias(a, b, bias=None):
    layout = image_layout(a)
    if layout is None or image_layout(b) != layout or not a.is_cuda or a.dtype != torch.float32:
        raise GqHipError("add_bias needs two dense fp32 HIP tensors of the same layout")
    B, C = a.shape[0], a.shape[1]
    HW = a.shape[2] * a.shape[3]
    y = torch.empty_like(a)
    with torch.cuda.device(a.device):
        _check(lib().add_bias_f32(a.data_ptr(), b.data_ptr(), _ptr(bias), y.data_ptr(), B, C, HW, layout, _stream()),
               "add_bias_f32")
    return y


def add_bias_stats(a, b, bias, groups: int):
    if image_layout(a) != 1 or image_layout(b) != 1 or not a.is_cuda or a.dtype != torch.float32 or not gn_nhwc_ok(a.shape[1], groups):
        raise GqHipError("add_bias_stats needs two dense channels_last fp32 HIP tensors with a GroupNorm-compatible C")
    B, C = a.shape[0], a.shape[1]
    HW = a.shape[2] * a.shape[3]
    y = torch.empty_like(a)
    stats = _stats_records(GNSTAT_WORDS * B * groups, a.device)
    with torch.cuda.device(a.device):
        _check(lib().add_bias_stats_f32(a.data_ptr(), b.data_ptr(), _ptr(bias), y.data_ptr(), B, C, HW, groups,
                                        stats.data_ptr(), _stream()), "add_bias_stats_f32")
    return y, stats


def gn_apply(x, gamma, beta, groups: int, eps: float, silu: bool, stats):
    if image_layout(x) != 1 or not x.is_cuda or x.dtype != torch.float32:
        raise GqHipError("gn_apply needs a dense channels_last fp32 HIP tensor")
    B, C = x.shape[0], x.shape[1]
    HW = x.shape[2] * x.shape[3]
    y = torch.empty_like(x)
    with torch.cuda.device(x.device):
        _check(lib().gn_apply_f32(x.data_ptr(), gamma.data_ptr(), beta.data_ptr(), y.data_ptr(), B, C, HW, groups,
                                  float(eps), 1 if silu else 0, stats.data_ptr(), _stream()), "gn_apply_f32")
    return y


def gn_stats_values(stats):
    r = stats.view(-1, GNSTAT_WORDS).double()
    s = (r[:, 2] * 2.0 ** 24 + r[:, 1] * 2.0 ** -16) + r[:, 0] * 2.0 ** -56
    ss = (r[:, 5] * 2.0 ** 24 + r[:, 4] * 2.0 ** -16) + r[:, 3] * 2.0 ** -56
    bad = r[:, 6] != 0
    s = torch.where(bad, torch.full_like(s, float("nan")), s)
    ss = torch.where(bad, torch.full_like(ss, float("nan")), ss)
    return torch.stack([s, ss], 1).flatten()


def gn_stats(x, groups: int, pre_bias=None):
    if image_layout(x) != 1 or not x.is_cuda or x.dtype != torch.float32 or not gn_nhwc_ok(x.shape[1], groups):
        raise GqHipError("gn_stats needs a dense channels_last fp32 HIP tensor with a GroupNorm-compatible C")
    B, C = x.shape[0], x.shape[1]
    stats = _stats_records(GNSTAT_WORDS * B * groups, x.device)
    with torch.cuda.device(x.device):
        _check(lib().gn_stats_f32(x.data_ptr(), _ptr(pre_bias), B, C, x.shape[2] * x.shape[3], groups, stats.data_ptr(),
                                  _stream()), "gn_stats_f32")
    return stats


def wino_conv3x3(x, U, gn=None, residual=None, bias=None, stats_groups: int = 0, f16=None):
    if image_layout(x) != 1 or not x.is_cuda or x.dtype != torch.float32 or x.shape[1] % 4 or x.shape[2] % 2 or x.shape[3] % 2:
        raise GqHipError("wino_conv3x3 needs a dense channels_last fp32 HIP tensor, C % 4 == 0, even H and W")
    B, C, H, W = x.shape
    cout = U.shape[2]
    f4 = U.shape[0] == 36
    if f4 and (H % 4 or W % 4):
        raise GqHipError("F(4x4,3x3) needs H, W multiples of 4")
    t = 4 if f4 else 2
    tiles = B * (H // t) * (W // t)
    L = lib()
    mscale = 1.0
    with torch.cuda.device(x.device):
        if f16 is not None:
            U3, u_scale, x_bound = f16[:3]
            amp = 100.0 if f4 else 4.0
            v_scale = 2.0 ** math.floor(math.log2(32768.0 / (amp * max(float(x_bound), 1e-30))))
            v_scale = min(v_scale, 2.0 ** 14)
            use_own = len(f16) > 3 and f16[3] is not None and tiles % 256 == 0 and own_gemm_fits(U.shape[0], tiles, cout, C)
            if use_own:
                V = torch.empty((U.shape[0], tiles, 2 * C), dtype=torch.float16, device=x.device)
                if gn is not None:
                    gamma, beta, groups, eps, silu, stats, pre_bias = gn
                    _check(L.wino_in_gn_nhwc_f16x2(x.data_ptr(), gamma.data_ptr(), beta.data_ptr(), _ptr(pre_bias),
                                                   stats.data_ptr(), V.data_ptr(), B, H, W, C, groups, float(eps),
                                                   1 if silu else 0, t, float(v_scale), _stream()), "wino_in_gn_nhwc_f16x2")
                else:
                    _check(L.wino_in_nhwc_f16x2(x.data_ptr(), V.data_ptr(), B, H, W, C, t, float(v_scale), _stream()),
                           "wino_in_nhwc_f16x2")
                M = torch.empty((U.shape[0], tiles, cout), dtype=torch.float32, device=x.device)
                _check(L.wino_gemm_f16x2(V.data_ptr(), f16[3].data_ptr(), M.data_ptr(), U.shape[0], tiles, C, cout,
                                         _stream()), "wino_gemm_f16x2")
                V = None
            else:
                V = torch.empty((U.shape[0], tiles, 3 * C), dtype=torch.float16, device=x.device)
            if V is None:
                pass
            elif gn is not None:
                gamma, beta, groups, eps, silu, stats, pre_bias = gn
                _check(L.wino_in_gn_nhwc_f16x3(x.data_ptr(), gamma.data_ptr(), beta.data_ptr(), _ptr(pre_bias),
                                               stats.data_ptr(), V.data_ptr(), B, H, W, C, groups, float(eps),
                                               1 if silu else 0, t, float(v_scale), _stream()), "wino_in_gn_nhwc_f16x3")
            else:
                _check(L.wino_in_nhwc_f16x3(x.data_ptr(), V.data_ptr(), B, H, W, C, t, float(v_scale), _stream()),
                       "wino_in_nhwc_f16x3")
            if V is not None:
                M = torch.bmm(V, U3, out_dtype=torch.float32)
            mscale = 1.0 / (v_scale * u_scale)
        else:
            V = torch.empty((U.shape[0], tiles, C), dtype=x.dtype, device=x.device)
            if gn is not None:
                gamma, beta, groups, eps, silu, stats, pre_bias = gn
                _check((L.wino4_in_gn_nhwc_f32 if f4 else L.wino_in_gn_nhwc_f32)(
                    x.data_ptr(), gamma.data_ptr(), beta.data_ptr(), _ptr(pre_bias), stats.data_ptr(), V.data_ptr(), B, H, W, C,
                    groups, float(eps), 1 if silu else 0, _stream()), "wino_in_gn_nhwc_f32")
            else:
                _check((L.wino4_in_nhwc_f32 if f4 else L.wino_in_nhwc_f32)(x.data_ptr(), V.data_ptr(), B, H, W, C, _stream()),
                       "wino_in_nhwc_f32")
            M = torch.bmm(V, U)
        y = torch.empty((B, cout, H, W), dtype=x.dtype, device=x.device, memory_format=torch.channels_last)
        if stats_groups:
            if (residual is not None and (image_layout(residual) != 1 or tuple(residual.shape) != tuple(y.shape))) \
                    or not gn_nhwc_ok(cout, stats_groups):
                raise GqHipError("fused Winograd tail needs a channels_last residual of the output shape and a GroupNorm-compatible C")
            stats = _stats_records(GNSTAT_WORDS * B * stats_groups, x.device)
            _check(L.wino_out_res_nhwc_f32(M.data_ptr(), _ptr(residual), _ptr(bias), y.data_ptr(), stats.data_ptr(),
                                           B, H, W, cout, stats_groups, t, float(mscale), _stream()), "wino_out_res_nhwc_f32")
            return y, stats
        _check((L.wino4_out_nhwc_f32 if f4 else L.wino_out_nhwc_f32)(M.data_ptr(), y.data_ptr(), B, H, W, cout,
                                                                     float(mscale), _stream()), "wino_out_nhwc_f32")
    return y


_BMM_OUT_DTYPE = None


def bmm_out_dtype_ok(device) -> bool:
    global _BMM_OUT_DTYPE
    if _BMM_OUT_DTYPE is None:
        try:
            a = torch.ones(1, 16, 16, dtype=torch.float16, device=device)
            _BMM_OUT_DTYPE = bool(torch.bmm(a, a, out_dtype=torch.float32).dtype == torch.float32)
        except (TypeError, RuntimeError):
            _BMM_OUT_DTYPE = False
    return _BMM_OUT_DTYPE


ATTN_L_OK = (64, 256, 1024, 2304, 4096)


def attention_f16x3(qkv, q_bound: float, v_bound: float):
    if not (qkv.is_cuda and qkv.dtype == torch.float32 and qkv.dim() == 3 and qkv.is_contiguous() and qkv.shape[2] % 12 == 0):
        raise GqHipError("attention_f16x3 needs a dense fp32 HIP tensor [B, L, 3C], C % 4 == 0")
    B, Ltok, C3 = qkv.shape
    C = C3 // 3
    if Ltok not in ATTN_L_OK:
        raise GqHipError("attention_f16x3: token count %d not in %s" % (Ltok, ATTN_L_OK))
    pow2 = lambda bound: min(2.0 ** math.floor(math.log2(32768.0 / max(float(bound), 1e-30))), 2.0 ** 14)
    sq, sv = pow2(q_bound), pow2(v_bound)
    L_ = lib()
    with torch.cuda.device(qkv.device):
        Q3 = torch.empty((B, Ltok, C3), dtype=torch.float16, device=qkv.device)
        K3 = torch.empty((B, Ltok, C3), dtype=torch.float16, device=qkv.device)
        V3 = torch.empty((B, 3 * Ltok, C), dtype=torch.float16, device=qkv.device)
        _check(L_.attn_split_qkv_f16x3(qkv.data_ptr(), Q3.data_ptr(), K3.data_ptr(), V3.data_ptr(), B, Ltok, C, sq, sv,
                                       _stream()), "attn_split_qkv_f16x3")
        S = torch.bmm(Q3, K3.transpose(1, 2), out_dtype=torch.float32)
        P3 = torch.empty((B, Ltok, 3 * Ltok), dtype=torch.float16, device=qkv.device)
        _check(L_.attn_softmax_split_f16x3(S.data_ptr(), P3.data_ptr(), B * Ltok, Ltok, float(C) ** -0.5 / (sq * sq), _stream()),
               "attn_softmax_split_f16x3")
        O = torch.bmm(P3, V3, out_dtype=torch.float32)
    return O, 1.0 / (16384.0 * sv)


def own_gemm_fits(positions: int, tiles: int, cout: int, cin: int = 256) -> bool:
    if cout % 256 == 0 and cin % 64 == 0:
        rounds = positions * (tiles // 256) * (cout // 256) / 256.0
    else:
        rounds = positions * (tiles // 256) * (cout // 128) / 512.0
    return rounds >= 1.0 and rounds / math.ceil(rounds) >= 0.85


def wino_weights_operand_order(h, l):
    T, cin, cout = h.shape
    planes = torch.stack([h, l], 0).reshape(2, T, cin // 16, 2, 8, cout // 32, 32)
    return planes.permute(1, 2, 5, 0, 3, 6, 4).reshape(T, cin // 16, cout // 32, 2, 64, 8).contiguous()


def conv3_weights_f16(weight):
    cout, cin, kk = weight.shape[0], weight.shape[1], weight.shape[2]
    if cout not in ((128, 256, 512, 1536) if kk == 1 else (128, 256)) or cin % 16 or tuple(weight.shape[2:]) not in ((3, 3), (1, 1)):
        raise GqHipError("conv3_weights_f16 needs a [128 | 256, Cin % 16 == 0, 3, 3] or [128 | 256 | 512 | 1536, Cin % 16 == 0, 1, 1] kernel")
    w = weight.detach().float()
    amax = float(w.abs().max())
    u_scale = 2.0 ** math.floor(math.log2(16384.0 / max(amax, 1e-30))) if amax > 0 else 1.0
    ws = w * u_scale
    hi = ws.half()
    lo = (ws - hi.float()).half()
    planes = torch.stack([hi, lo], 0)
    p7 = planes.reshape(2, cout // 32, 32, cin // 16, 2, 8, kk, kk).permute(3, 6, 7, 1, 0, 4, 2, 5)
    return p7.reshape(cin // 16, kk * kk, cout // 32, 2, 64, 8).contiguous(), u_scale


def conv3x3_direct(x, wf, u_scale: float, x_bound: float, gn, residual=None, bias=None, stats_groups: int = 0):
    if (image_layout(x) != 1 or not x.is_cuda or x.dtype != torch.float32 or x.shape[1] % 32 or x.shape[1] > 512 or x.shape[2] % 8
            or x.shape[3] % 32 or gn is None):
        raise GqHipError("conv3x3_direct needs a dense channels_last fp32 HIP tensor, C % 32 == 0, C <= 512, H % 8 == 0, W % 32 == 0, "
                         "and the GroupNorm that feeds the convolution")
    B, C, H, W = x.shape
    cout = wf.shape[2] * 32
    if wf.shape[0] * 16 != C:
        raise GqHipError("conv3x3_direct: weights are for %d input channels, x has %d" % (wf.shape[0] * 16, C))
    if residual is not None and (image_layout(residual) != 1 or tuple(residual.shape) != (B, cout, H, W)):
        raise GqHipError("conv3x3_direct: residual must be channels_last [B, Cout, H, W]")
    v_scale = min(2.0 ** math.floor(math.log2(32768.0 / max(float(x_bound), 1e-30))), 2.0 ** 14)
    L = lib()
    with torch.cuda.device(x.device):
        y = torch.empty((B, cout, H, W), dtype=x.dtype, device=x.device, memory_format=torch.channels_last)
        ostats = _stats_records(GNSTAT_WORDS * B * stats_groups, x.device) if stats_groups else None
        mscale = 1.0 / (v_scale * u_scale)
        gamma, beta, groups, eps, silu, stats, pre_bias = gn
        _check(L.conv3x3_gn_f16x3(x.data_ptr(), gamma.data_ptr(), beta.data_ptr(), _ptr(pre_bias), stats.data_ptr(),
                                  groups, float(eps), 1 if silu else 0, float(v_scale), wf.data_ptr(), _ptr(bias),
                                  _ptr(residual), y.data_ptr(), _ptr(ostats), B, H, W, C, cout, max(stats_groups, 1),
                                  mscale, _stream()), "conv3x3_gn_f16x3")
    return (y, ostats) if stats_groups else y


def conv1x1_direct(x, wf, u_scale: float, scale, residual=None, bias=None, stats_groups: int = 0, pre_bias=None,
                   post_scale: float = 1.0):
    if image_layout(x) != 1 or not x.is_cuda or x.dtype != torch.float32 or x.shape[1] % 32 or (x.shape[2] * x.shape[3]) % 256:
        raise GqHipError("conv1x1_direct needs a dense channels_last fp32 HIP tensor, C % 32 == 0, H * W % 256 == 0")
    B, C, H, W = x.shape
    cout = wf.shape[2] * 32
    if wf.shape[0] * 16 != C or wf.shape[1] != 1:
        raise GqHipError("conv1x1_direct: weights do not match (need conv3_weights_f16 of a [Cout, %d, 1, 1] kernel)" % C)
    if residual is not None and (image_layout(residual) != 1 or tuple(residual.shape) != (B, cout, H, W)):
        raise GqHipError("conv1x1_direct: residual must be channels_last [B, Cout, H, W]")
    if torch.is_tensor(scale):
        if post_scale != 1.0:
            raise GqHipError("conv1x1_direct: post_scale needs a host-side scale bound")
        sdev, v_scale, mscale = scale.data_ptr(), 0.0, 0.0
    else:
        v_scale = min(2.0 ** math.floor(math.log2(32768.0 / max(float(scale), 1e-30))), 2.0 ** 14)
        sdev, mscale = None, float(post_scale) / (v_scale * u_scale)
    with torch.cuda.device(x.device):
        y = torch.empty((B, cout, H, W), dtype=x.dtype, device=x.device, memory_format=torch.channels_last)
        ostats = _stats_records(GNSTAT_WORDS * B * stats_groups, x.device) if stats_groups else None
        _check(lib().conv1x1_f16x3(x.data_ptr(), _ptr(pre_bias), wf.data_ptr(), sdev, float(v_scale), float(mscale), _ptr(bias), _ptr(residual),
                                   y.data_ptr(), _ptr(ostats), B, H * W, C, cout, max(stats_groups, 1), _stream()),
               "conv1x1_f16x3")
    return (y, ostats) if stats_groups else y


def conv3s2_weights_f16(weight):
    cout, cin = weight.shape[0], weight.shape[1]
    if cout not in (128, 256, 512) or cin % 16 or tuple(weight.shape[2:]) != (3, 3):
        raise GqHipError("conv3s2_weights_f16 needs a [128 | 256 | 512, Cin % 16 == 0, 3, 3] kernel")
    w = weight.detach().float()
    amax = float(w.abs().max())
    u_scale = 2.0 ** math.floor(math.log2(16384.0 / max(amax, 1e-30))) if amax > 0 else 1.0
    ws = w * u_scale
    hi = ws.half()
    lo = (ws - hi.float()).half()
    planes = torch.stack([hi, lo], 0)
    std = planes.reshape(2, cout // 32, 32, cin // 16, 2, 8, 3, 3).permute(3, 6, 7, 1, 0, 4, 2, 5)
    steps = []
    for a, b in ((0, 0), (0, 1), (1, 0), (1, 1)):
        taps = [(dy, dx) for dy in range(2 if a == 0 else 1) for dx in range(2 if b == 0 else 1)]
        for chunk in range(cin // 16):
            for dy, dx in taps:
                steps.append(std[chunk, 2 * dy + a, 2 * dx + b])
    return torch.stack(steps, 0).reshape(9 * (cin // 16), cout // 32, 2, 64, 8).contiguous(), u_scale


def conv3x3s2_direct(x, wf, u_scale: float, scale, bias=None, stats_groups: int = 0):
    if image_layout(x) != 1 or not x.is_cuda or x.dtype != torch.float32 or x.shape[1] % 16 or x.shape[2] % 16 or x.shape[3] % 64:
        raise GqHipError("conv3x3s2_direct needs a dense channels_last fp32 HIP tensor, C % 16 == 0, H % 16 == 0, W % 64 == 0")
    B, C, H, W = x.shape
    cout = wf.shape[1] * 32
    if wf.shape[0] != 9 * (C // 16):
        raise GqHipError("conv3x3s2_direct: weights do not match the input channels")
    if torch.is_tensor(scale):
        sdev, v_scale, mscale = scale.data_ptr(), 0.0, 0.0
    else:
        v_scale = min(2.0 ** math.floor(math.log2(32768.0 / max(float(scale), 1e-30))), 2.0 ** 14)
        sdev, mscale = None, 1.0 / (v_scale * u_scale)
    with torch.cuda.device(x.device):
        y = torch.empty((B, cout, H // 2, W // 2), dtype=x.dtype, device=x.device, memory_format=torch.channels_last)
        ostats = _stats_records(GNSTAT_WORDS * B * stats_groups, x.device) if stats_groups else None
        _check(lib().conv3x3s2_f16x3(x.data_ptr(), wf.data_ptr(), sdev, float(v_scale), float(mscale), _ptr(bias), y.data_ptr(),
                                     _ptr(ostats), B, H, W, C, cout, max(stats_groups, 1), _stream()), "conv3x3s2_f16x3")
    return (y, ostats) if stats_groups else y


def upconv_weights_f16(phase_matrix, cin: int, cout: int):
    if cout not in (128, 256, 512) or cin % 16 or tuple(phase_matrix.shape) != (4 * cin, 4 * cout):
        raise GqHipError("upconv_weights_f16 needs the [4 Cin, 4 Cout] phase matrix, Cin % 16 == 0, Cout in (128, 256, 512)")
    w = phase_matrix.detach().float()
    amax = float(w.abs().max())
    u_scale = 2.0 ** math.floor(math.log2(16384.0 / max(amax, 1e-30))) if amax > 0 else 1.0
    ws = w * u_scale
    hi = ws.half()
    lo = (ws - hi.float()).half()
    planes = torch.stack([hi, lo], 0).reshape(2, 4, cin // 16, 2, 8, 4, cout // 32, 32)
    wf = planes.permute(5, 2, 1, 6, 0, 3, 7, 4).reshape(4, 4 * (cin // 16), cout // 32, 2, 64, 8)
    return wf.contiguous(), u_scale


def upconv2x_direct(x, wf, u_scale: float, scale, bias=None, stats_groups: int = 0):
    if image_layout(x) != 1 or not x.is_cuda or x.dtype != torch.float32 or x.shape[1] % 16 or x.shape[2] % 8 or x.shape[3] % 32:
        raise GqHipError("upconv2x_direct needs a dense channels_last fp32 HIP tensor, C % 16 == 0, H % 8 == 0, W % 32 == 0")
    B, C, H, W = x.shape
    cout = wf.shape[2] * 32
    if wf.shape[0] != 4 or wf.shape[1] != 4 * (C // 16):
        raise GqHipError("upconv2x_direct: weights do not match the input channels")
    if torch.is_tensor(scale):
        sdev, v_scale, mscale = scale.data_ptr(), 0.0, 0.0
    else:
        v_scale = min(2.0 ** math.floor(math.log2(32768.0 / max(float(scale), 1e-30))), 2.0 ** 14)
        sdev, mscale = None, 1.0 / (v_scale * u_scale)
    with torch.cuda.device(x.device):
        y = torch.empty((B, cout, 2 * H, 2 * W), dtype=x.dtype, device=x.device, memory_format=torch.channels_last)
        ostats = _stats_records(GNSTAT_WORDS * B * stats_groups, x.device) if stats_groups else None
        _check(lib().upconv2x_f16x3(x.data_ptr(), wf.data_ptr(), sdev, float(v_scale), float(mscale), _ptr(bias), y.data_ptr(),
                                    _ptr(ostats), B, H, W, C, cout, max(stats_groups, 1), _stream()), "upconv2x_f16x3")
    return (y, ostats) if stats_groups else y


def conv3x3_gn_small(x, w_ohwi, bias, gn):
    if image_layout(x) != 1 or not x.is_cuda or x.dtype != torch.float32 or x.shape[1] % 32 or x.shape[2] % 16 or x.shape[3] % 16:
        raise GqHipError("conv3x3_gn_small needs a dense channels_last fp32 HIP tensor, C % 32 == 0, H % 16 == 0, W % 16 == 0")
    B, C, H, W = x.shape
    cout = w_ohwi.shape[0]
    if tuple(w_ohwi.shape) != (cout, 3, 3, C) or not w_ohwi.is_contiguous() or w_ohwi.dtype != torch.float32:
        raise GqHipError("conv3x3_gn_small: weights must be fp32 [Cout, 3, 3, Cin] contiguous")
    gamma, beta, groups, eps, silu, stats, pre_bias = gn
    y = torch.empty((B, cout, H, W), dtype=x.dtype, device=x.device, memory_format=torch.channels_last)
    with torch.cuda.device(x.device):
        _check(lib().conv3x3_gn_small_f32(x.data_ptr(), gamma.data_ptr(), beta.data_ptr(), _ptr(pre_bias), stats.data_ptr(),
                                          groups, float(eps), 1 if silu else 0, w_ohwi.data_ptr(), _ptr(bias), y.data_ptr(),
                                          B, H, W, C, cout, _stream()), "conv3x3_gn_small_f32")
    return y


def checksum_table(tensors):
    dev = tensors[0].device
    rows = []
    for t in tensors:
        if not (t.is_cuda and t.element_size() == 4 and t.data_ptr() % 16 == 0 and t.device == dev):
            raise GqHipError("checksum_table needs 16-byte aligned 4-byte-element tensors on one HIP device")
        rows += [t.data_ptr(), t.numel()]
    return torch.tensor(rows, dtype=torch.int64).to(dev)


def checksum_tensors(table, out):
    with torch.cuda.device(table.device):
        _check(lib().gqhip_checksum_tensors(table.data_ptr(), table.numel() // 2, out.data_ptr(), _stream()), "gqhip_checksum_tensors")
    return out


def conv_f32_ok(cin: int, cout: int, H: int, W: int, gn: bool) -> bool:
    return cout % 4 == 0 and (cin % 64 == 0 and (not gn or cin <= 1024) or (not gn and cin in (8, 16, 32)))


def conv_f32_weights(weight):
    cout, cin = weight.shape[0], weight.shape[1]
    if cin % 8 or tuple(weight.shape[2:]) != (3, 3):
        raise GqHipError("conv_f32_weights needs a [Cout, Cin % 8 == 0, 3, 3] weight")
    nt = (cout + 31) // 32
    w = weight.detach().float().reshape(cout, cin, 9)
    if nt * 32 != cout:
        w = torch.cat([w, w.new_zeros(nt * 32 - cout, cin, 9)], 0)
    return w.reshape(nt, 32, cin // 8, 2, 4, 9).permute(0, 5, 2, 3, 1, 4).contiguous()


def conv3x3_f32(x, wk, cout: int, bias=None, gn=None):
    if image_layout(x) != 1 or not x.is_cuda or x.dtype != torch.float32:
        raise GqHipError("conv3x3_f32 needs a dense channels_last fp32 HIP tensor")
    B, C, H, W = x.shape
    if not conv_f32_ok(C, cout, H, W, gn is not None) or wk.numel() != ((cout + 31) // 32) * 9 * (C // 8) * 256:
        raise GqHipError(f"conv3x3_f32: shape {tuple(x.shape)} -> {cout} channels is not tiled by the kernel")
    y = torch.empty((B, cout, H, W), dtype=x.dtype, device=x.device, memory_format=torch.channels_last)
    gamma = beta = stats = pre_bias = None
    groups, eps, silu = 1, 0.0, False
    if gn is not None:
        gamma, beta, groups, eps, silu, stats, pre_bias = gn
    with torch.cuda.device(x.device):
        _check(lib().conv3x3_f32(x.data_ptr(), _ptr(gamma), _ptr(beta), _ptr(pre_bias), _ptr(stats), groups, float(eps),
                                 1 if silu else 0, wk.data_ptr(), _ptr(bias), y.data_ptr(), B, H, W, C, cout, _stream()),
               "conv3x3_f32")
    return y


def conv_cin_small_ok(cin: int, cout: int, H: int, W: int) -> bool:
    return 1 <= cin <= 4 and cout == 128 and H % 8 == 0 and W % 32 == 0 and H >= 8 and W >= 32


def conv_cin_small_weights(weight):
    cout, cin = weight.shape[0], weight.shape[1]
    return weight.detach().float().permute(2, 3, 1, 0).reshape(9 * cin, cout).contiguous()


def conv3x3_cin_small(x, wk, bias=None, stats_groups: int = 0):
    if image_layout(x) != 1 or not x.is_cuda or x.dtype != torch.float32:
# ... 208 lines not shown
```

vq-vae-from-gaussian-vae_amd/pit_hip/modules/unet.py:

```python
from __future__ import annotations

import math
import os

from typing import Sequence

import torch
import torch.nn as nn
import torch.nn.functional as F


def _gn(ch: int) -> nn.GroupNorm:
    return nn.GroupNorm(32, ch, eps=1e-6, affine=True)


def _silu(x: torch.Tensor) -> torch.Tensor:
    return F.silu(x)


def _use_fused(x: torch.Tensor, norm: nn.GroupNorm) -> bool:
    if not (FUSED_GN and x.is_cuda and x.dtype == torch.float32 and not torch.is_grad_enabled()
            and x.dim() == 4 and norm.affine):
        return False
    from .. import _lib
# ... 246 lines not shown
        wf2 = None
        if WINOGRAD_OWN_GEMM and U.shape[1] % 32 == 0 and U.shape[2] % 128 == 0:
            from .. import _lib

            wf2 = _lib.wino_weights_operand_order(h, l)
        return torch.cat([h, l, h], 1).contiguous(), u_scale, wf2

    return _cached(conv, "wino_u3", _wkey(conv.weight) + (f4, WINOGRAD_OWN_GEMM), build)


def _gn_act_bound(norm: nn.GroupNorm, x: torch.Tensor) -> float:
    gb = _cached(norm, "gb_max", _wkey(norm.weight, norm.bias),
                 lambda: (float(norm.weight.detach().abs().max()), float(norm.bias.detach().abs().max())))
    n = (x.shape[1] // norm.num_groups) * x.shape[2] * x.shape[3]
    return math.sqrt(max(n - 1, 1)) * gb[0] + gb[1]


class _WeightGuard:

    def __init__(self) -> None:
        self.key = None

    def begin(self, module: nn.Module) -> bool:
        from .. import _lib

        params = [p for p in module.parameters()]
        dense = lambda p: p.is_contiguous() or (p.dim() == 4 and p.is_contiguous(memory_format=torch.channels_last))
        if not params or not all(p.is_cuda and p.dtype == torch.float32 and dense(p) for p in params):
            return False
        key = tuple(p.data_ptr() for p in params)
        if key != self.key:
            try:
                self.table = _lib.checksum_table([p.detach() for p in params])
            except _lib.GqHipError:
                return False
            self.sums = torch.empty(len(params), dtype=torch.int64, device=params[0].device)
            self.host = torch.empty(len(params), dtype=torch.int64).pin_memory()
            self.event = torch.cuda.Event()
            self.baseline = None
            self.key = key
        self.versions = tuple(p._version for p in params)
        _lib.checksum_tensors(self.table, self.sums)
        self.host.copy_(self.sums, non_blocking=True)
        self.event.record()
        return True

    def changed(self) -> bool:
        self.event.synchronize()
        cur = self.host.clone()
        base, base_v = self.baseline, getattr(self, "baseline_versions", None)
        self.baseline, self.baseline_versions = cur, self.versions
        if base is None or torch.equal(cur, base):
            return False
        moved = (cur != base).tolist()
        return any(m and v == bv for m, v, bv in zip(moved, self.versions, base_v))


def _with_stats_arena(module: nn.Module, run, x: torch.Tensor):
    if not (STATS_ARENA and FUSED_GN and x.is_cuda and not torch.is_grad_enabled()) or torch.cuda.is_current_stream_capturing():
        return run(x)
    import threading

    from .. import _lib

    key = (threading.get_ident(), torch.cuda.current_stream(x.device).cuda_stream)
    arenas = module.__dict__.setdefault("_gq_stats_arenas", {})
    arena = arenas.pop(key, None)
    if arena is None:
        arena = _lib.StatsArena()
        module.__dict__.setdefault("_gq_stats_arena", arena)
        while len(arenas) >= _MAX_STATS_ARENAS:
            arenas.pop(next(iter(arenas)))
    arenas[key] = arena
    with _lib.stats_arena(arena, x.device):
        return run(x)


_MAX_STATS_ARENAS = 8


def _guarded(module: nn.Module, run0, x: torch.Tensor):
    run = lambda t: _with_stats_arena(module, run0, t)
    if not (WEIGHT_GUARD and getattr(module, "weight_guard", True) and x.is_cuda and not torch.is_grad_enabled()
            and not torch.cuda.is_current_stream_capturing()):
        return run(x)
    guard = module.__dict__.get("_gq_guard")
    if guard is None:
        guard = module.__dict__["_gq_guard"] = _WeightGuard()
    if not guard.begin(module):
        return run(x)
    y = run(x)
    if guard.changed():
        invalidate_caches(module)
        y = run(x)
    return y


def invalidate_caches(module: nn.Module) -> None:
    for m in module.modules():
        m.__dict__.pop("_gq_cache", None)


def _drop_caches_after_load(module, incompatible_keys) -> None:
    invalidate_caches(module)


def mark_winograd(module: nn.Module, f4: bool = False) -> None:
    for m in module.modules():
        if (isinstance(m, nn.Conv2d) and m.kernel_size == (3, 3) and m.stride == (1, 1) and m.padding == (1, 1)
                and m.dilation == (1, 1) and m.groups == 1 and m.padding_mode == "zeros"):
            m._gq_wino = True
            m._gq_wino4 = f4


def _add(a: torch.Tensor, b: torch.Tensor, bias=None) -> torch.Tensor:
    if (bias is not None and a.is_cuda and a.shape == b.shape and a.dtype == torch.float32
            and not torch.is_grad_enabled()):
        from .. import _lib

        la, lb = _lib.image_layout(a), _lib.image_layout(b)
        if FUSED_ADD_STATS and la == 1 and lb == 1 and _lib.gn_nhwc_ok(a.shape[1], GN_GROUPS):
            y, stats = _lib.add_bias_stats(a, b, bias, GN_GROUPS)
            y._gn_stats = (stats, GN_GROUPS)
            return y
        if la is not None and la == lb and ((la == 0 and (a.shape[2] * a.shape[3]) % 4 == 0) or
                                            (la == 1 and a.shape[1] % 4 == 0)):
            return _lib.add_bias(a, b, bias)
    return _materialize(a + b, bias)


FUSED_GN = True
WINOGRAD = True
WINOGRAD_MIN_CH = 128
FUSED_WINO_TAIL = True
WINOGRAD_F4 = True
WINOGRAD_F16X3 = True
WINOGRAD_OWN_GEMM = True
DIRECT_CONV = True
DIRECT_CONV_S2 = True
DIRECT_CONV_1X1 = True
FUSED_CONV_OUT = True
CONV_F32 = True
WEIGHT_GUARD = os.environ.get("GQHIP_WEIGHT_GUARD", "1") != "0"
FUSED_WINO_GN = True
FUSED_WINO_GN_F4 = True
WINOGRAD_ENCODER = True
DIRECT_UPCONV = True
FUSED_QKV = True
FUSED_ADD_STATS = True
STATS_ARENA = True
CONV_IN_SMALL = True
GN_GROUPS = 32
DEFER_BIAS = True
ATTN_F16X3 = True
ATTN_MATH = "auto"


def _sdpa(q, k, v):
    if ATTN_MATH is True or (ATTN_MATH == "auto" and q.is_cuda):
        w = torch.softmax(torch.matmul(q, k.transpose(-1, -2)) * (q.shape[-1] ** -0.5), dim=-1)
        return torch.matmul(w, v)
    return F.scaled_dot_product_attention(q, k, v)


def _conv3(cin: int, cout: int, padding_mode: str = "zeros", stride: int = 1, padding: int = 1) -> nn.Conv2d:
    return nn.Conv2d(cin, cout, 3, stride, padding, padding_mode=padding_mode)


class ResnetBlock(nn.Module):

    def __init__(self, cin: int, cout: int, dropout: float = 0.0, padding_mode: str = "zeros") -> None:
        super().__init__()
        self.in_channels, self.out_channels = cin, cout
        self.norm1 = _gn(cin)
        self.conv1 = _conv3(cin, cout, padding_mode)
        self.norm2 = _gn(cout)
        self.dropout = nn.Dropout(dropout)
        self.conv2 = _conv3(cout, cout, padding_mode)
        if cin != cout:
            self.nin_shortcut = nn.Conv2d(cin, cout, 1)

    def forward(self, x: torch.Tensor, pre_bias=None) -> torch.Tensor:
        h, b1 = _norm_act_conv(self.norm1, self.conv1, x, pre_bias, want_stats=True)
        if self.in_channels != self.out_channels and _pointwise_ok(self.nin_shortcut, x) and _use_fused(x, self.norm1):
            from .. import _lib

            wf, us = _direct_weights(self.nin_shortcut)
            scales = _lib.f16_scales(_stats_of(x, pre_bias, GN_GROUPS), 1.0, us)
            xs, bs = _lib.conv1x1_direct(x, wf, us, scales, pre_bias=pre_bias), self.nin_shortcut.bias
        elif self.in_channels != self.out_channels:
            xs, bs = _conv(self.nin_shortcut, x)
            if pre_bias is not None:
                wpb = self.nin_shortcut.weight.reshape(self.out_channels, self.in_channels) @ pre_bias
                bs = wpb if bs is None else bs + wpb
        else:
            xs, bs = x, pre_bias
        if self.dropout.p > 0.0 and self.training:
            h, bias = _conv(self.conv2, self.dropout(_norm_act(self.norm2, h, pre_bias=b1)))
        else:
            if (FUSED_WINO_TAIL and _defer_ok(h, self.conv2) and _wino_ok(self.conv2, h) and _use_fused(h, self.norm2)
                    and xs.shape[1] == self.out_channels and xs.is_contiguous(memory_format=torch.channels_last)
                    and not xs.is_contiguous()):
                from .. import _lib

                if (_direct_ok(self.conv2, h) and _lib.gn_nhwc_ok(self.out_channels, GN_GROUPS)
                        and _lib.image_layout(h) == 1):
                    bias = self.conv2.bias if bs is None else self.conv2.bias + bs
                    wf, us = _direct_weights(self.conv2)
                    y, ostats = _lib.conv3x3_direct(h, wf, us, _gn_act_bound(self.norm2, h),
                                                    gn=_gn_tuple(self.norm2, h, b1), residual=xs, bias=bias,
                                                    stats_groups=GN_GROUPS)
                    y._gn_stats = (ostats, GN_GROUPS)
                    return y
                if _lib.gn_nhwc_ok(self.out_channels, GN_GROUPS) and _lib.image_layout(h) == 1:
                    bias = self.conv2.bias if bs is None else self.conv2.bias + bs
                    f4 = (WINOGRAD_F4 and getattr(self.conv2, "_gq_wino4", False) and h.shape[2] % 4 == 0
                          and h.shape[3] % 4 == 0)
                    if FUSED_WINO_GN_F4 if f4 else FUSED_WINO_GN:
                        st = getattr(h, "_gn_stats", None)
                        if st is not None and b1 is None and st[1] == self.norm2.num_groups:
                            stats = st[0]
                        else:
                            stats = _lib.gn_stats(h, self.norm2.num_groups, b1)
                        gn = (self.norm2.weight, self.norm2.bias, self.norm2.num_groups, self.norm2.eps, True, stats, b1)
                        src = h
                        f16 = _f16_args_gn(self.conv2, self.norm2, h, f4)
                    else:
                        gn, src = None, _norm_act(self.norm2, h, pre_bias=b1)
                        f16 = _f16_args(self.conv2, src, f4)
                    y, ostats = _lib.wino_conv3x3(src, _wino_weights(self.conv2, f4), gn=gn, residual=xs, bias=bias,
                                                  stats_groups=GN_GROUPS, f16=f16)
                    y._gn_stats = (ostats, GN_GROUPS)
                    return y
            h, bias = _conv(self.conv2, _norm_act(self.norm2, h, pre_bias=b1))
        if bs is not None:
            bias = bs if bias is None else bias + bs
        return _add(xs, h, bias)


class AttnBlock(nn.Module):

    def __init__(self, ch: int) -> None:
        super().__init__()
        self.norm = _gn(ch)
        self.q = nn.Conv2d(ch, ch, 1)
        self.k = nn.Conv2d(ch, ch, 1)
        self.v = nn.Conv2d(ch, ch, 1)
        self.proj_out = nn.Conv2d(ch, ch, 1)

    def _qkv_weights(self):
        ps = (self.q.weight, self.k.weight, self.v.weight, self.q.bias, self.k.bias, self.v.bias)

        def build():
            c = self.q.weight.shape[0]
            return (torch.cat([p.detach().reshape(c, c) for p in ps[:3]], 0).t().contiguous(),
                    torch.cat([p.detach() for p in ps[3:]], 0).contiguous())

        return _cached(self, "qkv", _wkey(*ps), build)

    def forward(self, x: torch.Tensor) -> torch.Tensor:
        b, c, h, w = x.shape
        a_scale = 1.0
        y = _norm_act(self.norm, x, act=False)
        if y.is_contiguous(memory_format=torch.channels_last) and not y.is_contiguous():
            if FUSED_QKV and y.is_cuda and y.dtype == torch.float32 and not torch.is_grad_enabled():
                wqkv, bqkv = self._qkv_weights()
                if DIRECT_CONV_1X1 and c == 512 and (h * w) % 256 == 0:
                    from .. import _lib

                    qkv_wf, qkv_us = _cached(self, "qkv_wf", _wkey(self.q.weight, self.k.weight, self.v.weight),
                                             lambda: _lib.conv3_weights_f16(wqkv.t().reshape(3 * c, c, 1, 1)))
                    qkv = _lib.conv1x1_direct(y, qkv_wf, qkv_us, _gn_act_bound(self.norm, x), bias=bqkv)
                    qkv = qkv.permute(0, 2, 3, 1).reshape(b, 1, h * w, 3 * c)
                else:
                    qkv = torch.addmm(bqkv, y.permute(0, 2, 3, 1).reshape(b * h * w, c), wqkv).view(b, 1, h * w, 3 * c)
                q, k, v = qkv[..., :c], qkv[..., c:2 * c], qkv[..., 2 * c:]
            else:
                qkv = None
                q, k, v = (f(y).permute(0, 2, 3, 1).reshape(b, 1, h * w, c) for f in (self.q, self.k, self.v))
            if ATTN_F16X3 and qkv is not None and qkv.is_contiguous() and c % 4 == 0 and _f16_gemm_ok(qkv):
                from .. import _lib

                if (h * w) in _lib.ATTN_L_OK:
                    yb = _gn_act_bound(self.norm, x)
                    a, a_scale = _lib.attention_f16x3(qkv.view(b, h * w, 3 * c), self._qk_bound(yb), self._v_bound(yb))
            if a_scale == 1.0:
                a = _sdpa(q, k, v)
            a = a.reshape(b, h, w, c).permute(0, 3, 1, 2)
        else:
            q, k, v = (f(y).reshape(b, 1, c, h * w).transpose(2, 3).contiguous() for f in (self.q, self.k, self.v))
            a = _sdpa(q, k, v)
            a = a.transpose(2, 3).reshape(b, c, h, w)
        if (_pointwise_ok(self.proj_out, a) and FUSED_ADD_STATS and x.is_contiguous(memory_format=torch.channels_last)
                and not x.is_contiguous() and self.proj_out.bias is not None):
            from .. import _lib

            if _lib.image_layout(a) == 1 and _lib.gn_nhwc_ok(c, GN_GROUPS):
                wf, us = _direct_weights(self.proj_out)
                out, st = _lib.conv1x1_direct(a, wf, us, self._v_bound(_gn_act_bound(self.norm, x)) / a_scale, residual=x,
                                              bias=self.proj_out.bias, stats_groups=GN_GROUPS, post_scale=a_scale)
                out._gn_stats = (st, GN_GROUPS)
                return out
        if a_scale != 1.0:
            a = a * a_scale
        p, pb = _conv(self.proj_out, a)
        return _add(x, p, pb)

    def _qk_bound(self, y_bound: float) -> float:
        ps = (self.q.weight, self.k.weight, self.q.bias, self.k.bias)

        def build():
            c = self.q.weight.shape[0]
            rs = max(float(self.q.weight.detach().reshape(c, -1).abs().sum(1).max()),
                     float(self.k.weight.detach().reshape(c, -1).abs().sum(1).max()))
            return rs, max(float(self.q.bias.detach().abs().max()), float(self.k.bias.detach().abs().max()))

        qkb = _cached(self, "qk_bound", _wkey(*ps), build)
        return y_bound * qkb[0] + qkb[1]

    def _v_bound(self, y_bound: float) -> float:
        def build():
            wv = self.v.weight.detach().reshape(self.v.weight.shape[0], -1)
            return float(wv.abs().sum(1).max()), float(self.v.bias.detach().abs().max())

        vb = _cached(self, "v_bound", _wkey(self.v.weight, self.v.bias), build)
        return y_bound * vb[0] + vb[1]


class Downsample(nn.Module):

    def __init__(self, ch: int, with_conv: bool = True, padding_mode: str = "zeros") -> None:
        super().__init__()
        self.with_conv = with_conv
        self.mode = "constant" if padding_mode == "zeros" else padding_mode
        if with_conv:
            self.conv = _conv3(ch, ch, stride=2, padding=0)

    def forward(self, x: torch.Tensor):
        if not self.with_conv:
            return F.avg_pool2d(x, 2, 2), None
        conv = self.conv
        if (DIRECT_CONV_S2 and self.mode == "constant" and FUSED_GN and x.is_cuda and x.dtype == torch.float32
                and not torch.is_grad_enabled() and conv.out_channels in (128, 256, 512) and conv.in_channels % 16 == 0
                and conv.bias is not None and x.dim() == 4 and x.shape[2] % 16 == 0 and x.shape[3] % 64 == 0
                and x.is_contiguous(memory_format=torch.channels_last) and not x.is_contiguous()):
            from .. import _lib

            if _lib.gn_nhwc_ok(x.shape[1], GN_GROUPS) and _lib.gn_nhwc_ok(conv.out_channels, GN_GROUPS):
                s2_wf, s2_us = _cached(conv, "s2_wf", _wkey(conv.weight), lambda: _lib.conv3s2_weights_f16(conv.weight))
                scales = _lib.f16_scales(_stats_of(x, None, GN_GROUPS), 1.0, s2_us)
                y, st = _lib.conv3x3s2_direct(x, s2_wf, s2_us, scales, bias=conv.bias, stats_groups=GN_GROUPS)
                y._gn_stats = (st, GN_GROUPS)
                return y, None
        if self.mode == "constant":
            x = F.pad(x, (0, 1, 0, 1), mode="constant", value=0)
        else:
            x = F.pad(x, (0, 1, 0, 1), mode=self.mode)
        return _conv(self.conv, x)


class Upsample(nn.Module):

    def __init__(self, ch: int, with_conv: bool = True, padding_mode: str = "zeros") -> None:
        super().__init__()
        self.with_conv = with_conv
        if with_conv:
            self.conv = _conv3(ch, ch, padding_mode)

    def _phase_weights(self) -> torch.Tensor:
        def build():
            w = self.conv.weight.detach()
            rows = (((0,), (1, 2)), ((0, 1), (2,)))
            cout, cin = w.shape[0], w.shape[1]
            m = w.new_zeros(2, 2, cin, 2, 2, cout)
            for a in range(2):
                for b in range(2):
                    for u in range(2):
                        for v in range(2):
                            for kh in rows[a][u]:
                                for kw in rows[b][v]:
                                    m[u, v, :, a, b, :] += w[:, :, kh, kw].t()
            return m.reshape(4 * cin, 4 * cout).contiguous()

        return _cached(self, "phase_w", _wkey(self.conv.weight), build)

    def forward(self, x: torch.Tensor):
        fast = (FUSED_GN and x.is_cuda and x.dtype == torch.float32 and not torch.is_grad_enabled()
                and x.shape[1] % 4 == 0 and x.is_contiguous(memory_format=torch.channels_last) and not x.is_contiguous())
        if (fast and DIRECT_UPCONV and self.with_conv and _defer_ok(x, self.conv) and self.conv.kernel_size == (3, 3)
                and self.conv.stride == (1, 1) and self.conv.padding == (1, 1)):
            from .. import _lib

            b, c, h, w = x.shape
            st = getattr(x, "_gn_stats", None)
            cout = self.conv.out_channels
            if (st is not None and cout in (128, 256, 512) and c % 16 == 0 and h % 8 == 0 and w % 32 == 0
                    and self.conv.bias is not None and _lib.gn_nhwc_ok(cout, GN_GROUPS)):
                wf, wf_us = _cached(self, "phase_wf", _wkey(self.conv.weight),
                                    lambda: _lib.upconv_weights_f16(self._phase_weights(), c, cout))
                scales = _lib.f16_scales(st[0], 1.0, wf_us)
                y, ostats = _lib.upconv2x_direct(x, wf, wf_us, scales, bias=self.conv.bias, stats_groups=GN_GROUPS)
                y._gn_stats = (ostats, GN_GROUPS)
                return y, None
        if fast:
            from .. import _lib

            x = _lib.upsample2x_nhwc(x)
        else:
            x = F.interpolate(x, scale_factor=2.0, mode="nearest")
        return _conv(self.conv, x) if self.with_conv else (x, None)


def _make_attn(ch: int, attn_type: str) -> nn.Module:
    if attn_type == "vanilla":
        return AttnBlock(ch)
    if attn_type == "none":
        return nn.Identity()
    raise NotImplementedError(f"attn_type={attn_type!r} is not on the SD3-UNet hot path (reference unet.py:291-314)")


class _Level(nn.Module):

    def __init__(self) -> None:
        super().__init__()
        self.block = nn.ModuleList()
        self.attn = nn.ModuleList()

    def run(self, h: torch.Tensor, pre_bias=None) -> torch.Tensor:
        has_attn = len(self.attn) > 0
        for i, blk in enumerate(self.block):
            h = blk(h, pre_bias if i == 0 else None)
            if has_attn:
                h = self.attn[i](h)
        return h


class _Mid(nn.Module):
    def __init__(self, ch: int, dropout: float, padding_mode: str) -> None:
        super().__init__()
        self.block_1 = ResnetBlock(ch, ch, dropout, padding_mode)
        self.block_2 = ResnetBlock(ch, ch, dropout, padding_mode)

    def forward(self, h: torch.Tensor, pre_bias=None) -> torch.Tensor:
        return self.block_2(self.block_1(h, pre_bias))


class Encoder(nn.Module):
    def __init__(self, *, ch: int, out_ch: int = 3, ch_mult: Sequence[int] = (1, 2, 4, 8), num_res_blocks: int,
                 attn_resolutions: Sequence[int], dropout: float = 0.0, resamp_with_conv: bool = True,
                 in_channels: int, resolution: int, z_channels: int, double_z: bool = True,
                 use_linear_attn: bool = False, attn_type: str = "vanilla", padding_mode: str = "zeros",
                 **ignore_kwargs) -> None:
        super().__init__()
        self.register_load_state_dict_post_hook(_drop_caches_after_load)
        if use_linear_attn:
            attn_type = "linear"
        self.ch, self.resolution, self.in_channels = ch, resolution, in_channels
        self.num_resolutions, self.num_res_blocks = len(ch_mult), num_res_blocks
        self.conv_in = _conv3(in_channels, ch, padding_mode)
# ... 102 lines not shown
```

Before: 494.4.

## Fuse GroupNorm and QKV split into direct 1x1 conv for attention

Extends the direct 1x1 conv kernel to apply GroupNorm affine in its A-load path and to write Q/K/V directly as the split fp16 hi/lo operands the f16x3 attention kernel consumes. This removes the separate normalize pass, the fp32 qkv tensor, and the attention operand preparation. It also adds a half-height tile variant (RR=2) picked from CU count and tail occupancy, with a two-pass stats combine in the epilogue. The cost is more template variants and more LDS for the affine tables, and the split path depends on new attention_from_operands helpers.

After: 500.3, median of 6. +1.2%, better.

```diff
diff --git a/include/gqhip.h b/include/gqhip.h
--- a/include/gqhip.h
+++ b/include/gqhip.h
@@ -147,6 +147,14 @@
 int conv1x1_f16x3(const float *x, const float *pre_bias_or_null, const void *Wf, const float *scales_dev_or_null, float scale,
                   float mscale, const float *bias_or_null, const float *res_or_null, float *y, gqhip_gnstat_t *stats_out_or_null, int64_t B, int64_t HW,
                   int64_t Cin, int64_t Cout, int64_t groups_out, void *stream);
+int conv1x1_gn_f16x3(const float *x, const float *gamma, const float *beta, const float *pre_bias_or_null,
+                     const gqhip_gnstat_t *stats_in, int64_t groups_in, double eps, const void *Wf, float scale, float mscale,
+                     const float *bias_or_null, const float *res_or_null, float *y, gqhip_gnstat_t *stats_out_or_null, int64_t B,
+                     int64_t HW, int64_t Cin, int64_t Cout, int64_t groups_out, void *stream);
+int conv1x1_qkv_split_f16x3(const float *x, const float *gamma_or_null, const float *beta_or_null, const float *pre_bias_or_null,
+                            const gqhip_gnstat_t *stats_in_or_null, int64_t groups_in, double eps, const void *Wf, float scale,
+                            float mscale, const float *bias_or_null, void *Q3, void *K3, void *V3, float sq, float sv, int64_t B,
+                            int64_t L, int64_t C, void *stream);
 int conv3x3s2_f16x3(const float *x, const void *Wf, const float *scales_dev_or_null, float scale, float mscale,
                     const float *bias_or_null, float *y, gqhip_gnstat_t *stats_out_or_null, int64_t B, int64_t Hin, int64_t Win,
                     int64_t Cin, int64_t Cout, int64_t groups_out, void *stream);
diff --git a/vq-vae-from-gaussian-vae_amd/csrc/gq_conv3.h b/vq-vae-from-gaussian-vae_amd/csrc/gq_conv3.h
--- a/vq-vae-from-gaussian-vae_amd/csrc/gq_conv3.h
+++ b/vq-vae-from-gaussian-vae_amd/csrc/gq_conv3.h
@@ -72,8 +72,8 @@
   }
 }
 
-template <int COUT>
-__device__ __forceinline__ void conv3_epilogue(const Conv3Params &p, const Conv3Tile &t, const f32x16 (&acc)[4][2], unsigned char *sA,
+template <int COUT, int RR>
+__device__ __forceinline__ void conv3_epilogue(const Conv3Params &p, const Conv3Tile &t, const f32x16 (&acc)[RR][2], unsigned char *sA,
                                                int64_t *red, int wave, int wm, int wn) {
   constexpr int cout = COUT;
   const int lane = __lane_id(), tid = wave * 64 + lane;
@@ -84,7 +84,7 @@
 #pragma unroll
     for (int e = 0; e < 4; ++e) pb[e] = p.bias[t.nb * 128 + n + e];
   }
-  const long o = ((t.b * p.H + t.y0 + 4 * wm) * p.W + t.x0 + (lane >> 4)) * cout + t.nb * 128 + n;
+  const long o = ((t.b * p.H + t.y0 + RR * wm) * p.W + t.x0 + (lane >> 4)) * cout + t.nb * 128 + n;
   const long slice = (long)p.W * cout;
   StatPartial st;
   if (!p.stats) {
@@ -92,9 +92,26 @@
     else epi_store<2, false>(acc, stage, lane, p.y, nullptr, o, slice, 4 * cout, p.mscale, pb, st);
     return;
   }
-  if (p.res) epi_store<3, true>(acc, stage, lane, p.y, p.res, o, slice, 4 * cout, p.mscale, pb, st);
-  else epi_store<2, true>(acc, stage, lane, p.y, nullptr, o, slice, 4 * cout, p.mscale, pb, st);
-  stat_partial_flush(red + kStatWords * (n / p.cpg), st);
+  if constexpr (RR == 4) {
+    if (p.res) epi_store<3, true>(acc, stage, lane, p.y, p.res, o, slice, 4 * cout, p.mscale, pb, st);
+    else epi_store<2, true>(acc, stage, lane, p.y, nullptr, o, slice, 4 * cout, p.mscale, pb, st);
+    stat_partial_flush(red + kStatWords * (n / p.cpg), st);
+  } else {
+    __shared__ double part[2 * 64 * 4];
+    double *mine = part + (wn * 64 + lane) * 4;
+    if (wm == 0) {
+      if (p.res) epi_store<3, true>(acc, stage, lane, p.y, p.res, o, slice, 4 * cout, p.mscale, pb, st);
+      else epi_store<2, true>(acc, stage, lane, p.y, nullptr, o, slice, 4 * cout, p.mscale, pb, st);
+      mine[0] = st.v0; mine[1] = st.s; mine[2] = st.ss; mine[3] = (double)st.n;
+    }
+    __syncthreads();
+    if (wm == 1) {
+      st.v0 = mine[0]; st.s = mine[1]; st.ss = mine[2]; st.n = (int)mine[3];
+      if (p.res) epi_store<3, true>(acc, stage, lane, p.y, p.res, o, slice, 4 * cout, p.mscale, pb, st);
+      else epi_store<2, true>(acc, stage, lane, p.y, nullptr, o, slice, 4 * cout, p.mscale, pb, st);
+      stat_partial_flush(red + kStatWords * (n / p.cpg), st);
+    }
+  }
   __syncthreads();
   const int gpb = 128 / p.cpg, groups = cout / p.cpg;
   if (tid < kStatWords * gpb) stat_flush_word(p.stats + kStatWords * (t.b * groups + t.nb * gpb) + tid, red[tid]);
@@ -260,35 +277,73 @@
   const float *scales_dev;
   float scale;
   int cin;
+  const float *gamma, *beta;
+  const int64_t *stats_in;
+  int cpg_in;
+  double eps;
+  _Float16 *Q3, *K3, *V3;
+  float sq, sv;
 };
 
-template <int COUT>
+template <int COUT, int RR, int GN, int SPLIT>
 __global__ __launch_bounds__(256, 2) void conv1x1_f16x3_kernel(const Conv1Params pp) {
   typedef _Float16 f16x4 __attribute__((ext_vector_type(4)));
+  static_assert(RR == 4 || RR == 2, "rows of 32 pixels per wave");
+  static_assert((SPLIT != 0) == (COUT == 0), "the split epilogue takes cout at run time");
   Conv3Params p = pp.c;
-  constexpr int kPlane = 256 * 32, kChunk = 2 * kPlane, kStage = 2 * kChunk;
+  constexpr int NI = 2 * RR;
+  constexpr int kPlane = 32 * NI * 32, kChunk = 2 * kPlane, kStage = 2 * kChunk;
+  static_assert(2 * kStage >= 4 * kEpiWaveBytes, "the epilogue stages through sA");
   __shared__ __attribute__((aligned(16))) unsigned char sA[2 * kStage];
   __shared__ int64_t red[kStatWords * 32];
+  __shared__ __attribute__((aligned(16))) float sAff[2][GN ? 512 : 4];
   const int tid = threadIdx.x, lane = tid & 63, wave = __builtin_amdgcn_readfirstlane(tid >> 6);
   const int c = lane & 31, h = lane >> 5, wm = wave >> 1, wn = wave & 1;
   Conv3Tile t;
   if (!conv3_tile(p, t)) return;
+  t.y0 = t.y0 / kC3TH * NI;
   red[tid] = 0;
   const float scale = pp.scales_dev ? pp.scales_dev[0] : pp.scale;
   if (pp.scales_dev) p.mscale = pp.scales_dev[1];
   const int cin = pp.cin, nst = cin / 32;
+  if constexpr (GN != 0) {
+    const int groups = cin / pp.cpg_in;
+    const double n = (double)pp.cpg_in * (double)p.H * 32.0;
+    for (int ch = tid; ch < cin; ch += 256) {
+      const int g = ch / pp.cpg_in;
+      double st_s, st_ss;
+      stat_load(pp.stats_in + kStatWords * (t.b * groups + g), st_s, st_ss);
+      const double mean = st_s / n;
+      double var = st_ss / n - mean * mean;
+      var = var > 0.0 ? var : 0.0;
+      const double rstd = 1.0 / sqrt(var + pp.eps);
+      const double pbk = pp.pre_bias ? (double)pp.pre_bias[ch] : 0.0;
+      sAff[0][ch] = (float)(rstd * (double)pp.gamma[ch]);
+      sAff[1][ch] = (float)((double)pp.beta[ch] + (pbk - mean) * rstd * (double)pp.gamma[ch]);
+    }
+  }
   const int w8 = tid & 7, r0 = tid >> 3;
   const float *xb = pp.x + ((t.b * p.H + t.y0) * 32L + r0) * cin + 4 * w8;
-  const float *pbp = pp.pre_bias ? pp.pre_bias + 4 * w8 : nullptr;
-  f32x4 pb4 = {0.f, 0.f, 0.f, 0.f};
+  const float *pbp = (GN == 0 && pp.pre_bias) ? pp.pre_bias + 4 * w8 : nullptr;
+  f32x4 pb4 = {0.f, 0.f, 0.f, 0.f}, a4 = pb4, sh4 = pb4;
   const int loff = (w8 >> 2) * kChunk + r0 * 32 + 16 * (((w8 >> 1) & 1) ^ ((r0 >> 3) & 1)) + 8 * (w8 & 1);
-  f32x4 st[8];
+  f32x4 st[NI];
   auto issue = [&](int stage) {
 #pragma unroll
-    for (int i = 0; i < 8; ++i) st[i] = *reinterpret_cast<const f32x4 *>(xb + (long)(32 * i) * cin + stage * 32);
+    for (int i = 0; i < NI; ++i) st[i] = *reinterpret_cast<const f32x4 *>(xb + (long)(32 * i) * cin + stage * 32);
+  };
+  auto affine = [&](int stage) {
+    if constexpr (GN != 0) {
+      a4 = *reinterpret_cast<const f32x4 *>(&sAff[0][stage * 32 + 4 * w8]);
+      sh4 = *reinterpret_cast<const f32x4 *>(&sAff[1][stage * 32 + 4 * w8]);
+    } else {
+      if (pbp) pb4 = *reinterpret_cast<const f32x4 *>(pbp + stage * 32);
+    }
   };
   auto convert = [&](int i, int buf) {
-    const f32x4 v = (st[i] + pb4) * scale;
+    f32x4 v;
+    if constexpr (GN != 0) v = gn_act<0>(st[i], a4, sh4) * scale;
+    else v = (st[i] + pb4) * scale;
     f16x4 hi, lo;
 #pragma unroll
     for (int e = 0; e < 4; ++e) {
@@ -299,9 +354,12 @@
     *reinterpret_cast<f16x4 *>(d) = hi;
     *reinterpret_cast<f16x4 *>(d + kPlane) = lo;
   };
-  f32x16 acc[4][2];
-  GQ_C3_ZERO_ACC(acc);
-  const int aoff = (4 * wm) * 1024 + c * 32 + 16 * (h ^ ((c >> 3) & 1));
+  f32x16 acc[RR][2];
+#pragma unroll
+  for (int rr = 0; rr < RR; ++rr)
+#pragma unroll
+    for (int j = 0; j < 2; ++j) acc[rr][j] = f32x16{0.f, 0.f, 0.f, 0.f, 0.f, 0.f, 0.f, 0.f, 0.f, 0.f, 0.f, 0.f, 0.f, 0.f, 0.f, 0.f};
+  const int aoff = (RR * wm) * 1024 + c * 32 + 16 * (h ^ ((c >> 3) & 1));
   const unsigned char *wbase = reinterpret_cast<const unsigned char *>(p.Wf) + (4 * t.nb + 2 * wn) * 128 * 16;
   const int wl = lane * 16;
   const long wstep = (long)p.nnb * (512 * 16);
@@ -313,7 +371,7 @@
   };
   auto kstep = [&](const unsigned char *A, const f16x8 (&bq)[4]) {
 #pragma unroll
-    for (int rr = 0; rr < 4; ++rr) {
+    for (int rr = 0; rr < RR; ++rr) {
       const f16x8 ah = *reinterpret_cast<const f16x8 *>(A + aoff + rr * 1024);
       const f16x8 al = *reinterpret_cast<const f16x8 *>(A + aoff + rr * 1024 + kPlane);
 #pragma unroll
@@ -327,9 +385,10 @@
   const int nks = 2 * nst;
   load_b(0, b0);
   issue(0);
-  if (pbp) pb4 = *reinterpret_cast<const f32x4 *>(pbp);
-#pragma unroll
-  for (int i = 0; i < 8; ++i) convert(i, 0);
+  if constexpr (GN != 0) __syncthreads();
+  affine(0);
+#pragma unroll
+  for (int i = 0; i < NI; ++i) convert(i, 0);
   __syncthreads();
   for (int s = 0; s < nst; ++s) {
     const bool more = s + 1 < nst;
@@ -342,14 +401,33 @@
     load_b(2 * s + 2 < nks ? 2 * s + 2 : nks - 1, b0);
     kstep(A + kChunk, b1);
     if (more) {
-      if (pbp) pb4 = *reinterpret_cast<const f32x4 *>(pbp + (s + 1) * 32);
-#pragma unroll
-      for (int i = 0; i < 8; ++i) convert(i, nbuf);
+      affine(s + 1);
+#pragma unroll
+      for (int i = 0; i < NI; ++i) convert(i, nbuf);
     }
     __builtin_amdgcn_sched_barrier(0);
     __syncthreads();
   }
-  conv3_epilogue<COUT>(p, t, acc, sA, red, wave, wm, wn);
+  if constexpr (SPLIT != 0) {
+    const int C = p.cout / 3, col = t.nb * 128, third = col / C;
+    const int n = wn * 64 + 4 * (lane & 15), cc = col - third * C + n;
+    const long L = (long)p.H * 32, tok = (long)(t.y0 + RR * wm) * 32 + (lane >> 4);
+    f32x4 pb = {0.f, 0.f, 0.f, 0.f};
+    if (p.bias) {
+#pragma unroll
+      for (int e = 0; e < 4; ++e) pb[e] = p.bias[col + n + e];
+    }
+    float *stage = reinterpret_cast<float *>(sA + wave * kEpiWaveBytes);
+    if (third < 2) {
+      _Float16 *dst = third == 0 ? pp.Q3 : pp.K3;
+      epi_store_split(acc, stage, lane, dst, (t.b * L + tok) * 3 * C + cc, 32L * 3 * C, 4L * 3 * C, (long)C, third == 0, p.mscale,
+                      pb, pp.sq);
+    } else {
+      epi_store_split(acc, stage, lane, pp.V3, (t.b * 3 * L + tok) * C + cc, 32L * C, 4L * C, L * C, false, p.mscale, pb, pp.sv);
+    }
+  } else {
+    conv3_epilogue<COUT>(p, t, acc, sA, red, wave, wm, wn);
+  }
 }
 
 struct Conv3S2Params {
diff --git a/vq-vae-from-gaussian-vae_amd/csrc/gq_epilogue.h b/vq-vae-from-gaussian-vae_amd/csrc/gq_epilogue.h
--- a/vq-vae-from-gaussian-vae_amd/csrc/gq_epilogue.h
+++ b/vq-vae-from-gaussian-vae_amd/csrc/gq_epilogue.h
@@ -25,11 +25,11 @@
   for (int i = 0; i < 8; ++i) out[i] = s[64 * i];
 }
 
-template <int MODE, bool STATS>
-__device__ __forceinline__ void epi_store(const f32x16 (&acc)[4][2], float *stage, int lane, float *y, const float *res,
+template <int MODE, bool STATS, int RR>
+__device__ __forceinline__ void epi_store(const f32x16 (&acc)[RR][2], float *stage, int lane, float *y, const float *res,
                                           long o, long slice, long step, float mscale, f32x4 bias, StatPartial &st) {
 #pragma unroll
-  for (int rr = 0; rr < 4; ++rr) {
+  for (int rr = 0; rr < RR; ++rr) {
     __builtin_amdgcn_sched_barrier(0);
     const long orr = o + rr * slice;
     f32x4 rv[8];
@@ -49,4 +49,36 @@
   }
 }
 
+template <int RR>
+__device__ __forceinline__ void epi_store_split(const f32x16 (&acc)[RR][2], float *stage, int lane, _Float16 *dst, long o,
+                                                long slice, long step, long plane, bool second_h, float mscale,
+                                                f32x4 bias, float s) {
+  typedef _Float16 f16x4 __attribute__((ext_vector_type(4)));
+#pragma unroll
+  for (int rr = 0; rr < RR; ++rr) {
+    __builtin_amdgcn_sched_barrier(0);
+    const long orr = o + rr * slice;
+    f32x4 v[8];
+    epi_transpose(acc[rr], stage, lane, v);
+#pragma unroll
+    for (int i = 0; i < 8; ++i) {
+      f32x4 w = v[i];
+      w = w * mscale + bias;
+      w = w + f32x4{0.f, 0.f, 0.f, 0.f};
+      f16x4 h, l;
+#pragma unroll
+      for (int e = 0; e < 4; ++e) {
+        float x = w[e] * s;
+        asm volatile("" : "+v"(x));
+        h[e] = (_Float16)x;
+        l[e] = (_Float16)(x - (float)h[e]);
+      }
+      _Float16 *d = dst + orr + i * step;
+      *reinterpret_cast<f16x4 *>(d) = h;
+      *reinterpret_cast<f16x4 *>(d + plane) = second_h ? h : l;
+      *reinterpret_cast<f16x4 *>(d + 2 * plane) = second_h ? l : h;
+    }
+  }
 }
+
+}
diff --git a/vq-vae-from-gaussian-vae_amd/csrc/gqhip_unet.hip b/vq-vae-from-gaussian-vae_amd/csrc/gqhip_unet.hip
--- a/vq-vae-from-gaussian-vae_amd/csrc/gqhip_unet.hip
+++ b/vq-vae-from-gaussian-vae_amd/csrc/gqhip_unet.hip
@@ -330,29 +330,113 @@
 }
 #endif
 
+static int conv1_tile_rows(int64_t B, int64_t HW, int64_t Cout) {
+  const char *knob = getenv("GQHIP_CONV1_TILE");
+  if (knob && !strcmp(knob, "128")) return 2;
+  if (knob && !strcmp(knob, "256")) return HW % 256 == 0 ? 4 : 0;
+  if (HW % 256 != 0) return 2;
+  static thread_local int cus_of[64];
+  int dev = 0;
+  if (hipGetDevice(&dev) != hipSuccess || dev < 0 || dev >= 64) return 4;
+  if (cus_of[dev] == 0) {
+    int n = 0;
+    if (hipDeviceGetAttribute(&n, hipDeviceAttributeMultiprocessorCount, dev) != hipSuccess || n < 1) return 4;
+    cus_of[dev] = n;
+  }
+  const int64_t slots = 2 * (int64_t)cus_of[dev], blocks = B * (HW / 256) * (Cout / 128);
+  if (blocks < slots) return 2;
+  const int64_t last = blocks % slots;
+  return (last != 0 && last * 100 < slots * 85) ? 2 : 4;
+}
+
+#define GQ_C1_LAUNCH(RR, GN)                                                                                             \
+  do {                                                                                                                   \
+    if (split) hipLaunchKernelGGL((conv1x1_f16x3_kernel<0, RR, GN, 1>), grid, dim3(256), 0, st, gp);                     \
+    else if (Cout == 128) hipLaunchKernelGGL((conv1x1_f16x3_kernel<128, RR, GN, 0>), grid, dim3(256), 0, st, gp);        \
+    else if (Cout == 256) hipLaunchKernelGGL((conv1x1_f16x3_kernel<256, RR, GN, 0>), grid, dim3(256), 0, st, gp);        \
+    else if (Cout == 512) hipLaunchKernelGGL((conv1x1_f16x3_kernel<512, RR, GN, 0>), grid, dim3(256), 0, st, gp);        \
+    else hipLaunchKernelGGL((conv1x1_f16x3_kernel<1536, RR, GN, 0>), grid, dim3(256), 0, st, gp);                        \
+  } while (0)
+
+static int conv1_launch(Conv1Params &gp, const void *Wf, float mscale, const float *bias, const float *res, float *y,
+                        int64_t *stats_out, int64_t B, int64_t HW, int64_t Cin, int64_t Cout, int64_t groups_out, void *stream) {
+  const bool split = gp.Q3 != nullptr, gn = gp.gamma != nullptr;
+  const int rows = conv1_tile_rows(B, HW, Cout);
+  if (rows == 0) return GQHIP_ERR_INVALID_ARG;
+  hipStream_t st = static_cast<hipStream_t>(stream);
+  if (stats_out && stats_zero(stats_out, sizeof(int64_t) * kStatWords * B * groups_out, st) != hipSuccess) return check_launch();
+  Conv3Params &cp = gp.c;
+  conv3_fill(cp, Wf, bias, res, y, stats_out, B, HW / 32, 32, Cin, Cout, groups_out, mscale);
+  cp.nch = (int)(Cin / 16);
+  cp.tiles_x = 1; cp.tiles_y = (int)(HW / (64 * rows));
+  cp.ntiles = (long)B * cp.tiles_y;
+  cp.tiles_per_xcd = (cp.ntiles + 7) / 8;
+  gp.cin = (int)Cin;
+  const dim3 grid((unsigned)(8 * cp.tiles_per_xcd * cp.nnb));
+  if (rows == 4) {
+    if (gn) GQ_C1_LAUNCH(4, 1); else GQ_C1_LAUNCH(4, 0);
+  } else {
+    if (gn) GQ_C1_LAUNCH(2, 1); else GQ_C1_LAUNCH(2, 0);
+  }
+#undef GQ_C1_LAUNCH
+  return check_launch();
+}
+
+static bool conv1_shape_ok(int64_t B, int64_t HW, int64_t Cin) {
+  return B >= 0 && HW >= 128 && HW % 128 == 0 && Cin >= 32 && Cin % 32 == 0 && HW <= (1 << 24);
+}
+
+static bool conv1_gn_ok(int64_t Cin, int64_t groups_in) {
+  return Cin <= 512 && groups_in >= 1 && Cin % groups_in == 0 && (Cin / groups_in) % 4 == 0;
+}
+
 int conv1x1_f16x3(const float *x, const float *pre_bias_or_null, const void *Wf, const float *scales_dev_or_null, float scale,
                   float mscale, const float *bias_or_null, const float *res_or_null, float *y, int64_t *stats_out_or_null, int64_t B, int64_t HW,
                   int64_t Cin, int64_t Cout, int64_t groups_out, void *stream) {
-  if (B < 0 || HW < 256 || HW % 256 != 0 || Cin < 32 || Cin % 32 != 0 || (Cout != 128 && Cout != 256 && Cout != 512 && Cout != 1536) ||
-      HW > (1 << 24) || (!scales_dev_or_null && !(scale > 0.f)))
+  if (!conv1_shape_ok(B, HW, Cin) || (Cout != 128 && Cout != 256 && Cout != 512 && Cout != 1536) ||
+      (!scales_dev_or_null && !(scale > 0.f)))
     return GQHIP_ERR_INVALID_ARG;
   if (stats_out_or_null && !conv3_groups_ok(Cout, groups_out)) return GQHIP_ERR_INVALID_ARG;
   if (B == 0) return GQHIP_OK;
   if (!x || !Wf || !y) return GQHIP_ERR_INVALID_ARG;
-  hipStream_t st = static_cast<hipStream_t>(stream);
-  if (stats_out_or_null && stats_zero(stats_out_or_null, sizeof(int64_t) * kStatWords * B * groups_out, st) != hipSuccess)
-    return check_launch();
   Conv1Params gp{};
-  Conv3Params &cp = gp.c;
-  conv3_fill(cp, Wf, bias_or_null, res_or_null, y, stats_out_or_null, B, HW / 32, 32, Cin, Cout, groups_out, mscale);
-  cp.nch = (int)(Cin / 16);
-  gp.x = x; gp.pre_bias = pre_bias_or_null; gp.scales_dev = scales_dev_or_null; gp.scale = scale; gp.cin = (int)Cin;
-  const dim3 grid((unsigned)(8 * cp.tiles_per_xcd * cp.nnb));
-  if (Cout == 128) hipLaunchKernelGGL(conv1x1_f16x3_kernel<128>, grid, dim3(256), 0, st, gp);
-  else if (Cout == 256) hipLaunchKernelGGL(conv1x1_f16x3_kernel<256>, grid, dim3(256), 0, st, gp);
-  else if (Cout == 512) hipLaunchKernelGGL(conv1x1_f16x3_kernel<512>, grid, dim3(256), 0, st, gp);
-  else hipLaunchKernelGGL(conv1x1_f16x3_kernel<1536>, grid, dim3(256), 0, st, gp);
-  return check_launch();
+  gp.x = x; gp.pre_bias = pre_bias_or_null; gp.scales_dev = scales_dev_or_null; gp.scale = scale;
+  return conv1_launch(gp, Wf, mscale, bias_or_null, res_or_null, y, stats_out_or_null, B, HW, Cin, Cout, groups_out, stream);
+}
+
+int conv1x1_gn_f16x3(const float *x, const float *gamma, const float *beta, const float *pre_bias_or_null,
+                     const int64_t *stats_in, int64_t groups_in, double eps, const void *Wf, float scale, float mscale,
+                     const float *bias_or_null, const float *res_or_null, float *y, int64_t *stats_out_or_null, int64_t B,
+                     int64_t HW, int64_t Cin, int64_t Cout, int64_t groups_out, void *stream) {
+  if (!conv1_shape_ok(B, HW, Cin) || !conv1_gn_ok(Cin, groups_in) || (Cout != 128 && Cout != 256 && Cout != 512 && Cout != 1536) ||
+      !(scale > 0.f))
+    return GQHIP_ERR_INVALID_ARG;
+  if (stats_out_or_null && !conv3_groups_ok(Cout, groups_out)) return GQHIP_ERR_INVALID_ARG;
+  if (B == 0) return GQHIP_OK;
+  if (!x || !gamma || !beta || !stats_in || !Wf || !y) return GQHIP_ERR_INVALID_ARG;
+  Conv1Params gp{};
+  gp.x = x; gp.pre_bias = pre_bias_or_null; gp.scale = scale;
+  gp.gamma = gamma; gp.beta = beta; gp.stats_in = stats_in; gp.cpg_in = (int)(Cin / groups_in); gp.eps = eps;
+  return conv1_launch(gp, Wf, mscale, bias_or_null, res_or_null, y, stats_out_or_null, B, HW, Cin, Cout, groups_out, stream);
+}
+
+int conv1x1_qkv_split_f16x3(const float *x, const float *gamma_or_null, const float *beta_or_null, const float *pre_bias_or_null,
+                            const int64_t *stats_in_or_null, int64_t groups_in, double eps, const void *Wf, float scale,
+                            float mscale, const float *bias_or_null, void *Q3, void *K3, void *V3, float sq, float sv, int64_t B,
+                            int64_t L, int64_t C, void *stream) {
+  if (!conv1_shape_ok(B, L, C) || C % 128 != 0 || !(scale > 0.f) || !(sq > 0.f) || !(sv > 0.f))
+    return GQHIP_ERR_INVALID_ARG;
+  if (gamma_or_null && !conv1_gn_ok(C, groups_in)) return GQHIP_ERR_INVALID_ARG;
+  if (B == 0) return GQHIP_OK;
+  if (!x || !Wf || !Q3 || !K3 || !V3 || (gamma_or_null && (!beta_or_null || !stats_in_or_null))) return GQHIP_ERR_INVALID_ARG;
+  Conv1Params gp{};
+  gp.x = x; gp.pre_bias = pre_bias_or_null; gp.scale = scale;
+  if (gamma_or_null) {
+    gp.gamma = gamma_or_null; gp.beta = beta_or_null; gp.stats_in = stats_in_or_null; gp.cpg_in = (int)(C / groups_in); gp.eps = eps;
+  }
+  gp.Q3 = static_cast<_Float16 *>(Q3); gp.K3 = static_cast<_Float16 *>(K3); gp.V3 = static_cast<_Float16 *>(V3);
+  gp.sq = sq; gp.sv = sv;
+  return conv1_launch(gp, Wf, mscale, bias_or_null, nullptr, nullptr, nullptr, B, L, C, 3 * C, 1, stream);
 }
 
 int conv3x3s2_f16x3(const float *x, const void *Wf, const float *scales_dev_or_null, float scale, float mscale,
diff --git a/vq-vae-from-gaussian-vae_amd/pit_hip/_lib.py b/vq-vae-from-gaussian-vae_amd/pit_hip/_lib.py
--- a/vq-vae-from-gaussian-vae_amd/pit_hip/_lib.py
+++ b/vq-vae-from-gaussian-vae_amd/pit_hip/_lib.py
@@ -82,6 +82,10 @@
                                          _vp, _vp, _vp, _vp, _i64, _i64, _i64, _i64, _i64, _i64, ctypes.c_float, _vp]),
     "conv1x1_f16x3": (ctypes.c_int, [_vp, _vp, _vp, _vp, ctypes.c_float, ctypes.c_float, _vp, _vp, _vp, _vp, _i64, _i64, _i64, _i64, _i64,
                                       _vp]),
+    "conv1x1_gn_f16x3": (ctypes.c_int, [_vp, _vp, _vp, _vp, _vp, _i64, ctypes.c_double, _vp, ctypes.c_float, ctypes.c_float, _vp, _vp,
+                                         _vp, _vp, _i64, _i64, _i64, _i64, _i64, _vp]),
+    "conv1x1_qkv_split_f16x3": (ctypes.c_int, [_vp, _vp, _vp, _vp, _vp, _i64, ctypes.c_double, _vp, ctypes.c_float, ctypes.c_float,
+                                                _vp, _vp, _vp, _vp, ctypes.c_float, ctypes.c_float, _i64, _i64, _i64, _vp]),
     "conv3x3s2_f16x3": (ctypes.c_int, [_vp, _vp, _vp, ctypes.c_float, ctypes.c_float, _vp, _vp, _vp, _i64, _i64, _i64, _i64, _i64,
                                         _i64, _vp]),
     "conv3x3_gn_small_f32": (ctypes.c_int, [_vp, _vp, _vp, _vp, _vp, _i64, ctypes.c_double, ctypes.c_int, _vp, _vp, _vp, _i64, _i64,
@@ -719,6 +723,32 @@
 ATTN_L_OK = (64, 256, 1024, 2304, 4096)
 
 
+def attention_scales(q_bound: float, v_bound: float):
+    pow2 = lambda bound: min(2.0 ** math.floor(math.log2(32768.0 / max(float(bound), 1e-30))), 2.0 ** 14)
+    return pow2(q_bound), pow2(v_bound)
+
+
+def attention_operands(B: int, Ltok: int, C: int, device):
+    return (torch.empty((B, Ltok, 3 * C), dtype=torch.float16, device=device),
+            torch.empty((B, Ltok, 3 * C), dtype=torch.float16, device=device),
+            torch.empty((B, 3 * Ltok, C), dtype=torch.float16, device=device))
+
+
+def attention_from_operands(Q3, K3, V3, sq: float, sv: float):
+    B, Ltok, C3 = Q3.shape
+    C = C3 // 3
+    if Ltok not in ATTN_L_OK:
+        raise GqHipError("attention_f16x3: token count %d not in %s" % (Ltok, ATTN_L_OK))
+    L_ = lib()
+    with torch.cuda.device(Q3.device):
+        S = torch.bmm(Q3, K3.transpose(1, 2), out_dtype=torch.float32)
+        P3 = torch.empty((B, Ltok, 3 * Ltok), dtype=torch.float16, device=Q3.device)
+        _check(L_.attn_softmax_split_f16x3(S.data_ptr(), P3.data_ptr(), B * Ltok, Ltok, float(C) ** -0.5 / (sq * sq), _stream()),
+               "attn_softmax_split_f16x3")
+        O = torch.bmm(P3, V3, out_dtype=torch.float32)
+    return O, 1.0 / (16384.0 * sv)
+
+
 def attention_f16x3(qkv, q_bound: float, v_bound: float):
     if not (qkv.is_cuda and qkv.dtype == torch.float32 and qkv.dim() == 3 and qkv.is_contiguous() and qkv.shape[2] % 12 == 0):
         raise GqHipError("attention_f16x3 needs a dense fp32 HIP tensor [B, L, 3C], C % 4 == 0")
@@ -726,21 +756,12 @@
     C = C3 // 3
     if Ltok not in ATTN_L_OK:
         raise GqHipError("attention_f16x3: token count %d not in %s" % (Ltok, ATTN_L_OK))
-    pow2 = lambda bound: min(2.0 ** math.floor(math.log2(32768.0 / max(float(bound), 1e-30))), 2.0 ** 14)
-    sq, sv = pow2(q_bound), pow2(v_bound)
-    L_ = lib()
+    sq, sv = attention_scales(q_bound, v_bound)
     with torch.cuda.device(qkv.device):
-        Q3 = torch.empty((B, Ltok, C3), dtype=torch.float16, device=qkv.device)
-        K3 = torch.empty((B, Ltok, C3), dtype=torch.float16, device=qkv.device)
-        V3 = torch.empty((B, 3 * Ltok, C), dtype=torch.float16, device=qkv.device)
-        _check(L_.attn_split_qkv_f16x3(qkv.data_ptr(), Q3.data_ptr(), K3.data_ptr(), V3.data_ptr(), B, Ltok, C, sq, sv,
-                                       _stream()), "attn_split_qkv_f16x3")
-        S = torch.bmm(Q3, K3.transpose(1, 2), out_dtype=torch.float32)
-        P3 = torch.empty((B, Ltok, 3 * Ltok), dtype=torch.float16, device=qkv.device)
-        _check(L_.attn_softmax_split_f16x3(S.data_ptr(), P3.data_ptr(), B * Ltok, Ltok, float(C) ** -0.5 / (sq * sq), _stream()),
-               "attn_softmax_split_f16x3")
-        O = torch.bmm(P3, V3, out_dtype=torch.float32)
-    return O, 1.0 / (16384.0 * sv)
+        Q3, K3, V3 = attention_operands(B, Ltok, C, qkv.device)
+        _check(lib().attn_split_qkv_f16x3(qkv.data_ptr(), Q3.data_ptr(), K3.data_ptr(), V3.data_ptr(), B, Ltok, C, sq, sv,
+                                          _stream()), "attn_split_qkv_f16x3")
+    return attention_from_operands(Q3, K3, V3, sq, sv)
 
 
 def own_gemm_fits(positions: int, tiles: int, cout: int, cin: int = 256) -> bool:
@@ -759,8 +780,8 @@
 
 def conv3_weights_f16(weight):
     cout, cin, kk = weight.shape[0], weight.shape[1], weight.shape[2]
-    if cout not in ((128, 256, 512, 1536) if kk == 1 else (128, 256)) or cin % 16 or tuple(weight.shape[2:]) not in ((3, 3), (1, 1)):
-        raise GqHipError("conv3_weights_f16 needs a [128 | 256, Cin % 16 == 0, 3, 3] or [128 | 256 | 512 | 1536, Cin % 16 == 0, 1, 1] kernel")
+    if (cout % 128 if kk == 1 else cout not in (128, 256)) or cin % 16 or tuple(weight.shape[2:]) not in ((3, 3), (1, 1)):
+        raise GqHipError("conv3_weights_f16 needs a [128 | 256, Cin % 16 == 0, 3, 3] or [Cout % 128 == 0, Cin % 16 == 0, 1, 1] kernel")
     w = weight.detach().float()
     amax = float(w.abs().max())
     u_scale = 2.0 ** math.floor(math.log2(16384.0 / max(amax, 1e-30))) if amax > 0 else 1.0
@@ -797,30 +818,62 @@
     return (y, ostats) if stats_groups else y
 
 
+def _conv1_args(x, wf, scale, gn, post_scale: float, what: str, pre_bias=None):
+    if image_layout(x) != 1 or not x.is_cuda or x.dtype != torch.float32 or x.shape[1] % 32 or (x.shape[2] * x.shape[3]) % 128:
+        raise GqHipError(what + " needs a dense channels_last fp32 HIP tensor, C % 32 == 0, H * W % 128 == 0")
+    if wf.shape[0] * 16 != x.shape[1] or wf.shape[1] != 1:
+        raise GqHipError(what + ": weights do not match (need conv3_weights_f16 of a [Cout, %d, 1, 1] kernel)" % x.shape[1])
+    if gn is not None and pre_bias is not None and pre_bias is not gn[6]:
+        raise GqHipError(what + ": with gn the pending bias is gn[6] (the one its statistics include); pre_bias differs from it")
+    if gn is not None and (torch.is_tensor(scale) or gn[4] or x.shape[1] > 512 or (x.shape[1] // gn[2]) % 4):
+        raise GqHipError(what + ": the GroupNorm variant needs a host-side bound, no SiLU, C <= 512 and 4 | channels per group")
+    if torch.is_tensor(scale):
+        if post_scale != 1.0:
+            raise GqHipError(what + ": post_scale needs a host-side scale bound")
+        return scale.data_ptr(), 0.0
+    return None, min(2.0 ** math.floor(math.log2(32768.0 / max(float(scale), 1e-30))), 2.0 ** 14)
+
+
 def conv1x1_direct(x, wf, u_scale: float, scale, residual=None, bias=None, stats_groups: int = 0, pre_bias=None,
-                   post_scale: float = 1.0):
-    if image_layout(x) != 1 or not x.is_cuda or x.dtype != torch.float32 or x.shape[1] % 32 or (x.shape[2] * x.shape[3]) % 256:
-        raise GqHipError("conv1x1_direct needs a dense channels_last fp32 HIP tensor, C % 32 == 0, H * W % 256 == 0")
+                   post_scale: float = 1.0, gn=None):
+    sdev, v_scale = _conv1_args(x, wf, scale, gn, post_scale, "conv1x1_direct", pre_bias)
     B, C, H, W = x.shape
     cout = wf.shape[2] * 32
-    if wf.shape[0] * 16 != C or wf.shape[1] != 1:
-        raise GqHipError("conv1x1_direct: weights do not match (need conv3_weights_f16 of a [Cout, %d, 1, 1] kernel)" % C)
     if residual is not None and (image_layout(residual) != 1 or tuple(residual.shape) != (B, cout, H, W)):
         raise GqHipError("conv1x1_direct: residual must be channels_last [B, Cout, H, W]")
-    if torch.is_tensor(scale):
-        if post_scale != 1.0:
-            raise GqHipError("conv1x1_direct: post_scale needs a host-side scale bound")
-        sdev, v_scale, mscale = scale.data_ptr(), 0.0, 0.0
-    else:
-        v_scale = min(2.0 ** math.floor(math.log2(32768.0 / max(float(scale), 1e-30))), 2.0 ** 14)
-        sdev, mscale = None, float(post_scale) / (v_scale * u_scale)
+    mscale = 0.0 if sdev is not None else float(post_scale) / (v_scale * u_scale)
     with torch.cuda.device(x.device):
         y = torch.empty((B, cout, H, W), dtype=x.dtype, device=x.device, memory_format=torch.channels_last)
         ostats = _stats_records(GNSTAT_WORDS * B * stats_groups, x.device) if stats_groups else None
-        _check(lib().conv1x1_f16x3(x.data_ptr(), _ptr(pre_bias), wf.data_ptr(), sdev, float(v_scale), float(mscale), _ptr(bias), _ptr(residual),
-                                   y.data_ptr(), _ptr(ostats), B, H * W, C, cout, max(stats_groups, 1), _stream()),
-               "conv1x1_f16x3")
+        if gn is not None:
+            gamma, beta, groups, eps, _, stats, gn_pb = gn
+            _check(lib().conv1x1_gn_f16x3(x.data_ptr(), gamma.data_ptr(), beta.data_ptr(), _ptr(gn_pb), stats.data_ptr(), groups,
+                                          float(eps), wf.data_ptr(), float(v_scale), float(mscale), _ptr(bias), _ptr(residual),
+                                          y.data_ptr(), _ptr(ostats), B, H * W, C, cout, max(stats_groups, 1), _stream()),
+                   "conv1x1_gn_f16x3")
+        else:
+            _check(lib().conv1x1_f16x3(x.data_ptr(), _ptr(pre_bias), wf.data_ptr(), sdev, float(v_scale), float(mscale), _ptr(bias),
+                                       _ptr(residual), y.data_ptr(), _ptr(ostats), B, H * W, C, cout, max(stats_groups, 1),
+                                       _stream()), "conv1x1_f16x3")
     return (y, ostats) if stats_groups else y
+
+
+def qkv_split_direct(x, wf, u_scale: float, scale: float, sq: float, sv: float, bias=None, pre_bias=None, gn=None, out=None):
+    _, v_scale = _conv1_args(x, wf, float(scale), gn, 1.0, "qkv_split_direct", pre_bias)
+    B, C, H, W = x.shape
+    if wf.shape[2] * 32 != 3 * C or C % 128:
+        raise GqHipError("qkv_split_direct: needs the [3C, C, 1, 1] projection, C % 128 == 0")
+    gamma, beta, groups, eps, _, stats, gn_pb = gn if gn is not None else (None, None, 1, 0.0, False, None, pre_bias)
+    with torch.cuda.device(x.device):
+        Q3, K3, V3 = attention_operands(B, H * W, C, x.device) if out is None else out
+        for t, shape in zip((Q3, K3, V3), ((B, H * W, 3 * C), (B, H * W, 3 * C), (B, 3 * H * W, C))):
+            if not (t.is_cuda and t.dtype == torch.float16 and tuple(t.shape) == shape and t.is_contiguous()):
+                raise GqHipError("qkv_split_direct: out must be dense fp16 [B, L, 3C], [B, L, 3C], [B, 3L, C]")
+        _check(lib().conv1x1_qkv_split_f16x3(x.data_ptr(), _ptr(gamma), _ptr(beta), _ptr(gn_pb), _ptr(stats), groups, float(eps),
+                                             wf.data_ptr(), float(v_scale), 1.0 / (v_scale * u_scale), _ptr(bias), Q3.data_ptr(),
+                                             K3.data_ptr(), V3.data_ptr(), float(sq), float(sv), B, H * W, C, _stream()),
+               "conv1x1_qkv_split_f16x3")
+    return Q3, K3, V3
 
 
 def conv3s2_weights_f16(weight):
diff --git a/vq-vae-from-gaussian-vae_amd/pit_hip/modules/unet.py b/vq-vae-from-gaussian-vae_amd/pit_hip/modules/unet.py
--- a/vq-vae-from-gaussian-vae_amd/pit_hip/modules/unet.py
+++ b/vq-vae-from-gaussian-vae_amd/pit_hip/modules/unet.py
@@ -422,6 +422,7 @@
 CONV_IN_SMALL = True
 GN_GROUPS = 32
 DEFER_BIAS = True
+ATTN_FUSED_PROJ = True
 ATTN_F16X3 = True
 ATTN_MATH = "auto"
 
@@ -530,12 +531,21 @@
 
     def forward(self, x: torch.Tensor) -> torch.Tensor:
         b, c, h, w = x.shape
+        fused = self._fused_proj_attention(x) if ATTN_FUSED_PROJ else None
+        if fused is not None:
+            a, a_scale = fused[0].reshape(b, h, w, c).permute(0, 3, 1, 2), fused[1]
+        else:
+            a, a_scale = self._attention(x)
+        return self._proj_out(x, a, a_scale)
+
+    def _attention(self, x: torch.Tensor):
+        b, c, h, w = x.shape
         a_scale = 1.0
         y = _norm_act(self.norm, x, act=False)
         if y.is_contiguous(memory_format=torch.channels_last) and not y.is_contiguous():
             if FUSED_QKV and y.is_cuda and y.dtype == torch.float32 and not torch.is_grad_enabled():
                 wqkv, bqkv = self._qkv_weights()
-                if DIRECT_CONV_1X1 and c == 512 and (h * w) % 256 == 0:
+                if self._own_qkv_ok(y):
                     from .. import _lib
 
                     qkv_wf, qkv_us = _cached(self, "qkv_wf", _wkey(self.q.weight, self.k.weight, self.v.weight),
@@ -548,10 +558,10 @@
             else:
                 qkv = None
                 q, k, v = (f(y).permute(0, 2, 3, 1).reshape(b, 1, h * w, c) for f in (self.q, self.k, self.v))
-            if ATTN_F16X3 and qkv is not None and qkv.is_contiguous() and c % 4 == 0 and _f16_gemm_ok(qkv):
+            if qkv is not None and qkv.is_contiguous():
                 from .. import _lib
 
-                if (h * w) in _lib.ATTN_L_OK:
+                if self._f16x3_attention_ok(y):
                     yb = _gn_act_bound(self.norm, x)
                     a, a_scale = _lib.attention_f16x3(qkv.view(b, h * w, 3 * c), self._qk_bound(yb), self._v_bound(yb))
             if a_scale == 1.0:
@@ -561,6 +571,10 @@
             q, k, v = (f(y).reshape(b, 1, c, h * w).transpose(2, 3).contiguous() for f in (self.q, self.k, self.v))
             a = _sdpa(q, k, v)
             a = a.transpose(2, 3).reshape(b, c, h, w)
+        return a, a_scale
+
+    def _proj_out(self, x: torch.Tensor, a: torch.Tensor, a_scale: float) -> torch.Tensor:
+        c = x.shape[1]
         if (_pointwise_ok(self.proj_out, a) and FUSED_ADD_STATS and x.is_contiguous(memory_format=torch.channels_last)
                 and not x.is_contiguous() and self.proj_out.bias is not None):
             from .. import _lib
@@ -575,6 +589,36 @@
             a = a * a_scale
         p, pb = _conv(self.proj_out, a)
         return _add(x, p, pb)
+
+    @staticmethod
+    def _own_qkv_ok(y: torch.Tensor) -> bool:
+        return (FUSED_QKV and DIRECT_CONV_1X1 and y.is_cuda and y.dtype == torch.float32 and not torch.is_grad_enabled()
+                and y.shape[1] == 512 and (y.shape[2] * y.shape[3]) % 256 == 0
+                and y.is_contiguous(memory_format=torch.channels_last) and not y.is_contiguous())
+
+    @staticmethod
+    def _f16x3_attention_ok(y: torch.Tensor) -> bool:
+        from .. import _lib
+
+        return ATTN_F16X3 and y.shape[1] % 4 == 0 and _f16_gemm_ok(y) and (y.shape[2] * y.shape[3]) in _lib.ATTN_L_OK
+
+    def _fused_proj_attention(self, x: torch.Tensor):
+        b, c, h, w = x.shape
+        if not (self._own_qkv_ok(x) and self._f16x3_attention_ok(x) and _use_fused(x, self.norm)):
+            return None
+        from .. import _lib
+
+        if not _lib.gn_nhwc_ok(c, self.norm.num_groups):
+            return None
+        wqkv, bqkv = self._qkv_weights()
+        qkv_wf, qkv_us = _cached(self, "qkv_wf", _wkey(self.q.weight, self.k.weight, self.v.weight),
+                                 lambda: _lib.conv3_weights_f16(wqkv.t().reshape(3 * c, c, 1, 1)))
+        yb = _gn_act_bound(self.norm, x)
+        sq, sv = _lib.attention_scales(self._qk_bound(yb), self._v_bound(yb))
+        gn = (self.norm.weight, self.norm.bias, self.norm.num_groups, self.norm.eps, False,
+              _stats_of(x, None, self.norm.num_groups), None)
+        q3, k3, v3 = _lib.qkv_split_direct(x, qkv_wf, qkv_us, yb, sq, sv, bias=bqkv, gn=gn)
+        return _lib.attention_from_operands(q3, k3, v3, sq, sv)
 
     def _qk_bound(self, y_bound: float) -> float:
         ps = (self.q.weight, self.k.weight, self.q.bias, self.k.bias)
```
